# colinsongf/keyword_spotting

Hardware: AMD Instinct MI355X
Metric: mel-frames/s (real-time 10 ms-hop audio streams sustained = value/100) (higher is better)
Workload: dtype f32

## Files before the change

keyword_spotting_amd/csrc/gru_device.h:

```cpp
#pragma once
#include <type_traits>

#include "kws_internal.h"

namespace kws {

typedef float f32x4 __attribute__((ext_vector_type(4)));

__device__ __forceinline__ f32x4 mfma4(float a, float b, f32x4 c) {
    return __builtin_amdgcn_mfma_f32_16x16x4f32(a, b, c, 0, 0, 0);
}
__device__ __forceinline__ float sigmoid_f(float x) {
    return __builtin_amdgcn_rcpf(1.0f + __expf(-x));
}
__device__ __forceinline__ float tanh_f(float x) {
    return 1.0f - 2.0f * __builtin_amdgcn_rcpf(1.0f + __expf(2.0f * x));
}
#define KWS_MFMA_A(acc, wa, bv) \
    asm volatile("v_mfma_f32_16x16x4_f32 %0, %1, %2, %0" : "+v"(acc) : "a"(wa), "v"(bv))
__device__ __forceinline__ void mfma_fence(f32x4& a, f32x4& b, f32x4& c, f32x4& d) {
    asm volatile("s_nop 15" : "+v"(a), "+v"(b), "+v"(c), "+v"(d));
}
__device__ __forceinline__ void mfma_fence(f32x4& a, f32x4& b) {
    asm volatile("s_nop 15" : "+v"(a), "+v"(b));
}
__device__ __forceinline__ void mfma_prefence(f32x4& a, f32x4& b, f32x4& c, f32x4& d) {
    asm volatile("s_nop 3" : "+v"(a), "+v"(b), "+v"(c), "+v"(d));
}
__device__ __forceinline__ void mfma_prefence(f32x4& a, f32x4& b) {
    asm volatile("s_nop 3" : "+v"(a), "+v"(b));
}
__device__ __forceinline__ f32x4 splat4(float v) { f32x4 r = {v, v, v, v}; return r; }
__device__ __forceinline__ float bitsel(unsigned m, float a, float b) {
    return __uint_as_float((__float_as_uint(a) & m) | (__float_as_uint(b) & ~m));
}
template <int I0, int I1, class F>
__device__ __forceinline__ void static_for(F&& f) {
    if constexpr (I0 < I1) {
        f(std::integral_constant<int, I0>{});
        static_for<I0 + 1, I1>(f);
    }
}
constexpr float kLog2e = 1.4426950408889634f;
typedef float f32x2 __attribute__((ext_vector_type(2)));
__device__ __forceinline__ f32x2 sigmoid2(f32x2 x) {
    const f32x2 t = x * -kLog2e;
    f32x2 e;
    e.x = __builtin_amdgcn_exp2f(t.x);
    e.y = __builtin_amdgcn_exp2f(t.y);
    const f32x2 d = e + 1.0f;
    f32x2 r;
    r.x = __builtin_amdgcn_rcpf(d.x);
    r.y = __builtin_amdgcn_rcpf(d.y);
#ifdef KWS_FAULT_INJECT
    r = r * 1.0078125f;
#endif
    return r;
}
__device__ __forceinline__ f32x2 tanh2(f32x2 x) {
    const f32x2 t = x * (2.0f * kLog2e);
    f32x2 e;
    e.x = __builtin_amdgcn_exp2f(t.x);
    e.y = __builtin_amdgcn_exp2f(t.y);
    const f32x2 d = e + 1.0f;
    f32x2 r;
    r.x = __builtin_amdgcn_rcpf(d.x);
    r.y = __builtin_amdgcn_rcpf(d.y);
    return r * -2.0f + 1.0f;
}
__device__ __forceinline__ f32x4 ld4(const float* p) { return *reinterpret_cast<const f32x4*>(p); }

__device__ __forceinline__ void lds_barrier() {
    asm volatile("s_waitcnt lgkmcnt(0)" ::: "memory");
    __builtin_amdgcn_s_barrier();
    asm volatile("" ::: "memory");
}
constexpr int kRingFrames = 16;
constexpr int xs_stride(int kcx) { return 4 * ((((kcx + 3) / 4) & 1) ? (kcx + 3) / 4 : (kcx + 3) / 4 + 1); }
struct EpilogueLds {
    float* pstage;
    float* lring;
    int* words;
    int* carry;
    int8_t* cwords;
};
constexpr size_t kEpilogueLdsBytes = (4 * 16 * 8 + kRingFrames * 16 * 8) * 4 + kRingFrames * 16 * 4 + 2 * 16 * 4;
__device__ __forceinline__ EpilogueLds epilogue_carve(char* base) {
    EpilogueLds e;
    e.pstage = reinterpret_cast<float*>(base);
    e.lring = e.pstage + 4 * 16 * 8;
    e.words = reinterpret_cast<int*>(e.lring + kRingFrames * 16 * 8);
    e.carry = e.words + kRingFrames * 16;
    e.cwords = nullptr;
    return e;
}

__device__ __forceinline__ void epilogue_fold(const EpilogueLds& e, int t, int lane) {
    if (lane < 32) {
        const int s = lane >> 1, half = lane & 1;
        f32x4 v = *reinterpret_cast<const f32x4*>(e.pstage + (0 * 16 + s) * 8 + 4 * half);
#pragma unroll
        for (int w = 1; w < 4; ++w) v += *reinterpret_cast<const f32x4*>(e.pstage + (w * 16 + s) * 8 + 4 * half);
        *reinterpret_cast<f32x4*>(e.lring + (((t & (kRingFrames - 1)) * 16 + s) * 8 + 4 * half)) = v;
    }
}

struct FoldRegs { f32x4 v[4]; };
__device__ __forceinline__ void epilogue_fold_load(const EpilogueLds& e, int lane, FoldRegs& r) {
    if (lane < 32) {
        const int s = lane >> 1, half = lane & 1;
#pragma unroll
        for (int w = 0; w < 4; ++w) r.v[w] = *reinterpret_cast<const f32x4*>(e.pstage + (w * 16 + s) * 8 + 4 * half);
    }
}
__device__ __forceinline__ void epilogue_fold_store(const EpilogueLds& e, int t, int lane, const FoldRegs& r) {
    if (lane < 32) {
        const int s = lane >> 1, half = lane & 1;
        const f32x4 v = ((r.v[0] + r.v[1]) + r.v[2]) + r.v[3];
        *reinterpret_cast<f32x4*>(e.lring + (((t & (kRingFrames - 1)) * 16 + s) * 8 + 4 * half)) = v;
    }
}

template <bool OPAQUE_LANE = false>
__device__ __forceinline__ void epilogue_flush(const GruLayerParams& p, const EpilogueLds& e, int group, int t0,
                                               int n, int w, int lane, bool final_flush) {
    if constexpr (OPAQUE_LANE) asm volatile("" : "+v"(lane));
    const int f = 4 * w + (lane & 3);
    const int s = lane >> 2;
    const int b = group * kStreamsPerGroup + s;
    const int C = p.C;
    float lg[kMaxClasses];
    {
        const f32x4* row = reinterpret_cast<const f32x4*>(e.lring + (f * 16 + s) * 8);
        const f32x4 lo = row[0], hi = row[1];
#pragma unroll
        for (int c = 0; c < 4; ++c) { lg[c] = lo[c]; lg[4 + c] = hi[c]; }
    }
    if (p.use_relu) {
#pragma unroll
        for (int c = 0; c < kMaxClasses; ++c) {
            lg[c] = fmaxf(lg[c], 0.f);
            if (p.value_clip > 0.f) lg[c] = fminf(lg[c], 20.f);
        }
    }
    float m = lg[0];
#pragma unroll
    for (int c = 1; c < kMaxClasses; ++c) m = (c < C) ? fmaxf(m, lg[c]) : m;
    float pr[kMaxClasses];
    float sum = 0.f;
#pragma unroll
    for (int c = 0; c < kMaxClasses; ++c) {
        pr[c] = (c < C) ? __expf(lg[c] - m) : 0.f;
        sum += pr[c];
    }
    const float inv = __builtin_amdgcn_rcpf(sum);
#pragma unroll
    for (int c = 0; c < kMaxClasses; ++c) pr[c] *= inv;
    int word = -1;
    float best = -1.f;
#pragma unroll
    for (int c = 1; c < kMaxClasses - 1; ++c) {
        if (c < C - 1 && pr[c] > best) { best = pr[c]; word = c - 1; }
    }
    if (!(best > p.decode_thres)) word = -1;
    e.words[f * 16 + s] = word;
    if (e.cwords != nullptr) {
        int ln = lane;
        asm volatile("" : "+v"(ln));
        const int f2 = 4 * w + (ln & 3);
        if (f2 < n) e.cwords[(ln >> 2) * kWinTailWordsStride + t0 + f2] = (int8_t)word;
    }
    const bool mine = b < p.B && f < n;
    const size_t row = (size_t)b * (p.t_stride ? p.t_stride : p.T) + (t0 + f);
    if (mine) {
        if (C == 6) {
            if (p.logits) {
                float2* o = reinterpret_cast<float2*>(p.logits + row * 6);
                o[0] = make_float2(lg[0], lg[1]); o[1] = make_float2(lg[2], lg[3]); o[2] = make_float2(lg[4], lg[5]);
            }
            if (p.softmax) {
                float2* o = reinterpret_cast<float2*>(p.softmax + row * 6);
                o[0] = make_float2(pr[0], pr[1]); o[1] = make_float2(pr[2], pr[3]); o[2] = make_float2(pr[4], pr[5]);
            }
        } else {
            if (p.logits) {
#pragma unroll
                for (int c = 0; c < kMaxClasses; ++c)
                    if (c < C) p.logits[row * C + c] = lg[c];
            }
            if (p.softmax) {
#pragma unroll
                for (int c = 0; c < kMaxClasses; ++c)
                    if (c < C) p.softmax[row * C + c] = pr[c];
            }
        }
    }
    lds_barrier();
    const int blk = (t0 / kRingFrames) & 1;
    const int prev = f == 0 ? e.carry[blk * 16 + s] : e.words[(f - 1) * 16 + s];
    const int token = (word >= 0 && word != prev) ? word + 1 : 0;
    if (f == n - 1) {
        if (!final_flush) e.carry[(blk ^ 1) * 16 + s] = word;
        else if (b < p.B && p.prev_word) p.prev_word[b] = word;
    }
    if (mine && p.tokens) p.tokens[row] = (int8_t)token;
}


}
```

keyword_spotting_amd/csrc/gru_kernels.hip:

```cpp
#include <cstddef>

#include "gru_device.h"
#include "launch.h"
#include "window_device.h"

namespace kws {

template <int KCX, bool FIRST, bool LAST, bool WINDOW = false>
__global__ void __launch_bounds__(256) __attribute__((amdgpu_waves_per_eu(1, 1)))
gru_layer_resident(const GruLayerParams p) {
    static_assert(!WINDOW || (LAST && !FIRST), "the window tail belongs to the last layer of a stack");
    constexpr int H = 128, NT = 8, KCH = 32;
    const int tid = threadIdx.x;
    const int w = __builtin_amdgcn_readfirstlane(tid >> 6);
    const int lane = tid & 63, g = lane >> 4, s = lane & 15;
    const int n_groups = (p.B + kStreamsPerGroup - 1) / kStreamsPerGroup;
    int group = blockIdx.x;
    int b_raw = group * kStreamsPerGroup + s;
    bool bvalid = b_raw < p.B;
    int b = bvalid ? b_raw : p.B - 1;
    const int T = p.T;
    const int n0 = 2 * w, n1 = 2 * w + 1;

    extern __shared__ __attribute__((aligned(16))) char smem[];
    f32x4* hbuf = reinterpret_cast<f32x4*>(smem);
    f32x4* rhbuf = hbuf + NT * 64;
    f32x4* wlds = rhbuf + NT * 64;
    EpilogueLds epi = epilogue_carve(reinterpret_cast<char*>(wlds + 4 * KCX * 64));
    if constexpr (WINDOW) epi.cwords = reinterpret_cast<int8_t*>(reinterpret_cast<char*>(wlds + 4 * KCX * 64) + kEpilogueLdsBytes);
    const uint8_t* win_dl = reinterpret_cast<const uint8_t*>(epi.cwords) + 16 * kWinTailWordsStride;
    constexpr size_t kWinOffset = offsetof(GruLayerParams, win);
    if constexpr (WINDOW) window_tail_prepare(window_tail_params_from_kernarg(kWinOffset), const_cast<uint8_t*>(win_dl), tid);
    constexpr int kXsStride = xs_stride(KCX);
    float* xs = reinterpret_cast<float*>(reinterpret_cast<char*>(wlds + 4 * KCX * 64) + (LAST ? kEpilogueLdsBytes : 0));

    float wgh[2][2][KCH];
    float wch[2][KCH];
    float wcx[2][KCX];
    const f32x4* wh4 = reinterpret_cast<const f32x4*>(p.wh);
#pragma unroll
    for (int j = 0; j < 2; ++j) {
        const int n = 2 * w + j;
#pragma unroll
        for (int k4 = 0; k4 < KCH / 4; ++k4) {
            const f32x4 vr = wh4[((n * 3 + 0) * (KCH / 4) + k4) * 64 + lane];
            const f32x4 vu = wh4[((n * 3 + 1) * (KCH / 4) + k4) * 64 + lane];
            const f32x4 vc = wh4[((n * 3 + 2) * (KCH / 4) + k4) * 64 + lane];
#pragma unroll
            for (int e = 0; e < 4; ++e) {
                wgh[j][0][4 * k4 + e] = vr[e];
                wgh[j][1][4 * k4 + e] = vu[e];
                wch[j][4 * k4 + e] = vc[e];
            }
        }
    }
    if constexpr (FIRST) {
#pragma unroll
        for (int j = 0; j < 2; ++j)
#pragma unroll
            for (int kc = 0; kc < KCX; ++kc) wcx[j][kc] = p.wx[(((2 * w + j) * 3 + 2) * KCX + kc) * 64 + lane];
        for (int kc = 0; kc < KCX; ++kc) {
            f32x4 v;
            v.x = p.wx[((n0 * 3 + 0) * KCX + kc) * 64 + lane];
            v.y = p.wx[((n0 * 3 + 1) * KCX + kc) * 64 + lane];
            v.z = p.wx[((n1 * 3 + 0) * KCX + kc) * 64 + lane];
            v.w = p.wx[((n1 * 3 + 1) * KCX + kc) * 64 + lane];
            wlds[(w * KCX + kc) * 64 + lane] = v;
        }
    } else {
        const f32x4* wx4 = reinterpret_cast<const f32x4*>(p.wx);
#pragma unroll
        for (int j = 0; j < 2; ++j)
#pragma unroll
            for (int k4 = 0; k4 < KCX / 4; ++k4) {
                const f32x4 vc = wx4[(((2 * w + j) * 3 + 2) * (KCX / 4) + k4) * 64 + lane];
#pragma unroll
                for (int e = 0; e < 4; ++e) wcx[j][4 * k4 + e] = vc[e];
            }
        for (int k4 = 0; k4 < KCX / 4; ++k4) {
            const f32x4 r0 = wx4[((n0 * 3 + 0) * (KCX / 4) + k4) * 64 + lane];
            const f32x4 u0 = wx4[((n0 * 3 + 1) * (KCX / 4) + k4) * 64 + lane];
            const f32x4 r1 = wx4[((n1 * 3 + 0) * (KCX / 4) + k4) * 64 + lane];
            const f32x4 u1 = wx4[((n1 * 3 + 1) * (KCX / 4) + k4) * 64 + lane];
#pragma unroll
            for (int e = 0; e < 4; ++e)
                wlds[(w * KCX + 4 * k4 + e) * 64 + lane] = (f32x4){r0[e], u0[e], r1[e], u1[e]};
        }
    }
#pragma unroll
    for (int j = 0; j < 2; ++j) {
#pragma unroll
        for (int kc = 0; kc < KCH; ++kc) {
            asm volatile("" : "+a"(wgh[j][0][kc]));
            asm volatile("" : "+a"(wgh[j][1][kc]));
            asm volatile("" : "+a"(wch[j][kc]));
        }
    }
    asm volatile("s_nop 7" ::: "memory");
    f32x4 bias_r[2], bias_u[2], bias_c[2];
#pragma unroll
    for (int j = 0; j < 2; ++j) {
        const int n = 2 * w + j;
        bias_r[j] = ld4(p.bias + 0 * H + n * 16 + 4 * g);
        bias_u[j] = ld4(p.bias + 1 * H + n * 16 + 4 * g);
        bias_c[j] = ld4(p.bias + 2 * H + n * 16 + 4 * g);
    }
    float wfc[2][4];
    f32x4 bfc4 = splat4(0.f);
    if (LAST) {
#pragma unroll
        for (int j = 0; j < 2; ++j)
#pragma unroll
            for (int e = 0; e < 4; ++e) wfc[j][e] = p.wfc[((2 * w + j) * 4 + e) * 64 + lane];
        if (w == 0) bfc4 = ld4(p.bfc + 4 * g);
    }

    int len_s = T;
    f32x4 hreg[2];
    const float4* xl_src = nullptr;
    const float4* xprev = nullptr;
    constexpr int XQ = KCX;
    const int xl_row = lane / XQ, xl_q = lane % XQ;
    const bool xl_active = FIRST && lane < 4 * XQ;
    auto enter_group = [&]() {
        b_raw = group * kStreamsPerGroup + s;
        bvalid = b_raw < p.B;
        b = bvalid ? b_raw : p.B - 1;
        const bool do_reset = p.reset != nullptr && p.reset[b] != 0;
        len_s = p.seq_len ? p.seq_len[b] - p.t_base : T;
#pragma unroll
        for (int j = 0; j < 2; ++j) {
            const int n = 2 * w + j;
            hreg[j] = do_reset ? splat4(0.f) : ld4(p.state_in + (size_t)b * H + n * 16 + 4 * g);
            hbuf[n * 64 + lane] = hreg[j];
        }
        if (LAST && tid < 16) {
            const int bb = group * kStreamsPerGroup + tid;
            int pw = -1;
            if (bb < p.B && p.prev_word && !(p.reset && p.reset[bb])) pw = p.prev_word[bb];
            epi.carry[tid] = pw;
        }
        if constexpr (FIRST) {
            const int xl_b = min(group * kStreamsPerGroup + 4 * w + (xl_active ? xl_row : 0), p.B - 1);
            xl_src = reinterpret_cast<const float4*>(p.x_mel + (size_t)xl_b * (p.t_stride ? p.t_stride : T) * p.I) + xl_q;
        } else {
            xprev = p.x_prev + (size_t)group * T * NT * 64 + lane;
        }
    };

    float4 xl_inflight = make_float4(0.f, 0.f, 0.f, 0.f);
    auto coop_issue = [&](int t_req) {
        const int t = t_req < T ? t_req : T - 1;
        if (xl_active) xl_inflight = xl_src[(size_t)t * XQ];
    };
    auto coop_commit = [&]() {
        if (xl_active) {
            float* dst = xs + (4 * (4 * w + xl_row)) * kXsStride + xl_q;
            dst[0 * kXsStride] = xl_inflight.x;
            dst[1 * kXsStride] = xl_inflight.y;
            dst[2 * kXsStride] = xl_inflight.z;
            dst[3 * kXsStride] = xl_inflight.w;
        }
    };
    float xbuf0[KCX];
    auto read_xs = [&](float (&dst)[KCX]) {
        const float* row = xs + (4 * s + g) * kXsStride;
#pragma unroll
        for (int k4 = 0; k4 < KCX / 4; ++k4) {
            const f32x4 v = *reinterpret_cast<const f32x4*>(row + 4 * k4);
            dst[4 * k4 + 0] = v[0]; dst[4 * k4 + 1] = v[1]; dst[4 * k4 + 2] = v[2]; dst[4 * k4 + 3] = v[3];
        }
        if constexpr (KCX % 4 >= 2) {
            const f32x2 v = *reinterpret_cast<const f32x2*>(row + (KCX / 4) * 4);
            dst[(KCX / 4) * 4 + 0] = v[0]; dst[(KCX / 4) * 4 + 1] = v[1];
        }
        if constexpr (KCX % 2 == 1) dst[KCX - 1] = row[KCX - 1];
    };
    auto load_x_slice = [&](float (&dst)[KCX], int t_req, const int sl) {
        if constexpr (!FIRST) {
            const int t = t_req < T ? t_req : T - 1;
            const float4 v = xprev[((size_t)t * NT + sl) * 64];
            dst[4 * sl + 0] = v.x; dst[4 * sl + 1] = v.y; dst[4 * sl + 2] = v.z; dst[4 * sl + 3] = v.w;
        }
    };

    f32x4 acc_r[2], acc_u[2], acc_c[2];
    auto gates_x_part = [&](const float (&xB)[KCX], auto k0_, auto k1_, auto pin_) {
        constexpr int K0 = decltype(k0_)::value, K1 = decltype(k1_)::value;
        constexpr bool PIN = decltype(pin_)::value;
        f32x4 ring[3];
        if (K0 < K1) ring[K0 % 3] = wlds[(w * KCX + K0) * 64 + lane];
        if (K0 + 1 < K1) ring[(K0 + 1) % 3] = wlds[(w * KCX + K0 + 1) * 64 + lane];
#pragma unroll
        for (int kc = K0; kc < K1; ++kc) {
            if (kc + 2 < K1) ring[(kc + 2) % 3] = wlds[(w * KCX + kc + 2) * 64 + lane];
            if (PIN) __builtin_amdgcn_sched_barrier(0);
            const f32x4 a4 = ring[kc % 3];
            acc_r[0] = mfma4(a4.x, xB[kc], acc_r[0]);
            acc_u[0] = mfma4(a4.y, xB[kc], acc_u[0]);
            acc_r[1] = mfma4(a4.z, xB[kc], acc_r[1]);
            acc_u[1] = mfma4(a4.w, xB[kc], acc_u[1]);
            if (PIN) __builtin_amdgcn_sched_barrier(0);
        }
    };
    using pinned = std::true_type;
    constexpr int KSPLIT = KCX / 2;
    using k_lo = std::integral_constant<int, 0>;
    using k_mid = std::integral_constant<int, KSPLIT>;
    using k_hi = std::integral_constant<int, KCX>;
    auto cand_x = [&](const float (&xB)[KCX]) {
#pragma unroll
        for (int j = 0; j < 2; ++j) acc_c[j] = bias_c[j];
#pragma unroll
        for (int kc = 0; kc < KCX; ++kc) {
            acc_c[0] = mfma4(wcx[0][kc], xB[kc], acc_c[0]);
            acc_c[1] = mfma4(wcx[1][kc], xB[kc], acc_c[1]);
        }
    };

    f32x4 hb_a, hb_b;

    auto frame = [&](int t, float (&xcur)[KCX], float (&xnxt)[KCX]) {
        mfma_prefence(acc_r[0], acc_u[0], acc_r[1], acc_u[1]);
#pragma unroll
        for (int nn = 0; nn < NT; ++nn) {
            const f32x4 hb = (nn & 1) ? hb_b : hb_a;
            if (nn + 2 < NT) {
                if (nn & 1) hb_b = hbuf[(nn + 2) * 64 + lane]; else hb_a = hbuf[(nn + 2) * 64 + lane];
            }
            if constexpr (FIRST) { if (nn == 0) coop_issue(t + 2); } else load_x_slice(xnxt, t + 1, nn);
            __builtin_amdgcn_sched_barrier(0);
#pragma unroll
            for (int e = 0; e < 4; ++e) {
                const int kc = 4 * nn + e;
                const float hv = hb[e];
                KWS_MFMA_A(acc_r[0], wgh[0][0][kc], hv);
                KWS_MFMA_A(acc_u[0], wgh[0][1][kc], hv);
                KWS_MFMA_A(acc_r[1], wgh[1][0][kc], hv);
                KWS_MFMA_A(acc_u[1], wgh[1][1][kc], hv);
            }
        }
        mfma_fence(acc_r[0], acc_u[0], acc_r[1], acc_u[1]);
        if constexpr (FIRST) read_xs(xcur);
        f32x4 u[2];
#pragma unroll
        for (int j = 0; j < 2; ++j) {
            const f32x2 r_lo = sigmoid2((f32x2){acc_r[j][0], acc_r[j][1]});
            const f32x2 r_hi = sigmoid2((f32x2){acc_r[j][2], acc_r[j][3]});
            const f32x2 rh_lo = r_lo * (f32x2){hreg[j][0], hreg[j][1]};
            const f32x2 rh_hi = r_hi * (f32x2){hreg[j][2], hreg[j][3]};
            rhbuf[(2 * w + j) * 64 + lane] = (f32x4){rh_lo.x, rh_lo.y, rh_hi.x, rh_hi.y};
        }
#pragma unroll
        for (int j = 0; j < 2; ++j) {
            const f32x2 u_lo = sigmoid2((f32x2){acc_u[j][0], acc_u[j][1]});
            const f32x2 u_hi = sigmoid2((f32x2){acc_u[j][2], acc_u[j][3]});
            u[j] = (f32x4){u_lo.x, u_lo.y, u_hi.x, u_hi.y};
        }
#pragma unroll
        for (int j = 0; j < 2; ++j) { acc_r[j] = bias_r[j]; acc_u[j] = bias_u[j]; }
        __builtin_amdgcn_sched_barrier(0);
        gates_x_part(xcur, k_lo{}, k_mid{}, pinned{});
        lds_barrier();
        hb_a = rhbuf[0 * 64 + lane];
        hb_b = rhbuf[1 * 64 + lane];
        gates_x_part(xcur, k_mid{}, k_hi{}, pinned{});

        mfma_prefence(acc_c[0], acc_c[1]);
#pragma unroll
        for (int nn = 0; nn < NT; ++nn) {
            const f32x4 rb = (nn & 1) ? hb_b : hb_a;
            if (nn + 2 < NT) {
                if (nn & 1) hb_b = rhbuf[(nn + 2) * 64 + lane]; else hb_a = rhbuf[(nn + 2) * 64 + lane];
            }
            __builtin_amdgcn_sched_barrier(0);
#pragma unroll
            for (int e = 0; e < 4; ++e) {
                const int kc = 4 * nn + e;
                const float rv = rb[e];
                KWS_MFMA_A(acc_c[0], wch[0][kc], rv);
                KWS_MFMA_A(acc_c[1], wch[1][kc], rv);
            }
        }
        mfma_fence(acc_c[0], acc_c[1]);
        const unsigned live = t < len_s ? 0xffffffffu : 0u;
        f32x4 hout[2];
#pragma unroll
        for (int j = 0; j < 2; ++j) {
#pragma unroll
            for (int h2 = 0; h2 < 2; ++h2) {
                const f32x2 c = tanh2((f32x2){acc_c[j][2 * h2], acc_c[j][2 * h2 + 1]});
                const f32x2 uu = {u[j][2 * h2], u[j][2 * h2 + 1]};
                const f32x2 hh = {hreg[j][2 * h2], hreg[j][2 * h2 + 1]};
                const f32x2 hn = (1.0f - uu) * c + uu * hh;
                hreg[j][2 * h2] = bitsel(live, hn.x, hh.x);
                hreg[j][2 * h2 + 1] = bitsel(live, hn.y, hh.y);
                if (LAST) {
                    hout[j][2 * h2] = bitsel(live, hn.x, 0.f);
                    hout[j][2 * h2 + 1] = bitsel(live, hn.y, 0.f);
                }
            }
        }
#pragma unroll
        for (int j = 0; j < 2; ++j) acc_c[j] = bias_c[j];
        constexpr int NCX = 2 * KCX;
        constexpr int NPOST = NCX >= 32 ? 16 : 8;
        constexpr int NPRE = NCX - NPOST;
        auto cand_x_mfma = [&](auto mc) {
            constexpr int m = decltype(mc)::value, kc = m / 2;
            if constexpr (m % 2 == 0) acc_c[0] = mfma4(wcx[0][kc], xcur[kc], acc_c[0]);
            else acc_c[1] = mfma4(wcx[1][kc], xcur[kc], acc_c[1]);
        };
        if constexpr (FIRST) coop_commit();
#pragma unroll
        for (int j = 0; j < 2; ++j) {
            hbuf[(2 * w + j) * 64 + lane] = hreg[j];
            if (!LAST) {
                const f32x4 o = hreg[j];
                p.h_out[((size_t)group * T + t) * NT * 64 + (2 * w + j) * 64 + lane] =
                    make_float4(o[0], o[1], o[2], o[3]);
            }
        }
        if (LAST) {
            f32x4 accf = bfc4;
#pragma unroll
            for (int j = 0; j < 2; ++j)
#pragma unroll
                for (int e = 0; e < 4; ++e) accf = mfma4(wfc[j][e], hout[j][e], accf);
            if (g < 2) *reinterpret_cast<f32x4*>(epi.pstage + (w * 16 + s) * 8 + 4 * g) = accf;
        }
        __builtin_amdgcn_sched_barrier(0);
        static_for<0, NPRE>(cand_x_mfma);
        __builtin_amdgcn_sched_barrier(0);
        lds_barrier();
        hb_a = hbuf[0 * 64 + lane];
        hb_b = hbuf[1 * 64 + lane];
        FoldRegs fold;
        const bool folder = LAST && w == (t & 3);
        if (folder) epilogue_fold_load(epi, lane, fold);
        __builtin_amdgcn_sched_barrier(0);
        static_for<NPRE, NCX>(cand_x_mfma);
        __builtin_amdgcn_sched_barrier(0);
        if (LAST) {
            if (folder) epilogue_fold_store(epi, t, lane, fold);
            if (((t + 1) & (kRingFrames - 1)) == 0 || t == T - 1) {
                const int t0 = t & ~(kRingFrames - 1);
                lds_barrier();
                epilogue_flush(p, epi, group, t0, t - t0 + 1, w, lane, t == T - 1);
            }
        }
    };

    for (; group < n_groups; group += gridDim.x) {
    enter_group();
    __syncthreads();
    if (T > 0) {
        if constexpr (FIRST) {
            coop_issue(0);
            coop_commit();
            __syncthreads();
            read_xs(xbuf0);
            coop_issue(1);
        } else {
#pragma unroll
            for (int sl = 0; sl < NT; ++sl) load_x_slice(xbuf0, 0, sl);
        }
#pragma unroll
        for (int j = 0; j < 2; ++j) { acc_r[j] = bias_r[j]; acc_u[j] = bias_u[j]; }
        gates_x_part(xbuf0, k_lo{}, k_hi{}, pinned{});
        hb_a = hbuf[0 * 64 + lane];
        hb_b = hbuf[1 * 64 + lane];
        cand_x(xbuf0);
        if constexpr (FIRST) {
            __syncthreads();
            coop_commit();
            __syncthreads();
        }
    }
    for (int t = 0; t < T; ++t) frame(t, xbuf0, xbuf0);

    if (bvalid) {
#pragma unroll
        for (int j = 0; j < 2; ++j)
            *reinterpret_cast<f32x4*>(p.state_out + (size_t)b * H + (2 * w + j) * 16 + 4 * g) = hreg[j];
    }
    __syncthreads();
    if constexpr (WINDOW) {
        const WindowTail win = window_tail_params_from_kernarg(kWinOffset);
        WindowTailRegs<2> wreq;
        window_tail_request<2>(win, p.B, group * kStreamsPerGroup, tid, wreq);
        window_tail<2>(win, p.B, group * kStreamsPerGroup, T, epi.cwords, kWinTailWordsStride, win_dl, reinterpret_cast<char*>(hbuf), tid, wreq);
        __syncthreads();
    }
    }
}

constexpr float kResidualScale = 0.7071067811865475f;
constexpr float kLayerNormEps = 1e-5f;

template <int TPW, bool FIRST, bool LAST, bool PIPE, bool WRAP = false>
__device__ __forceinline__ void gru_layer_generic_body(const GruLayerParams& p, const int group,
                                                       const GruWrapLayer& wl = GruWrapLayer{nullptr, 0.f, 0}) {
    constexpr int NT = 4 * TPW, H = 64 * TPW;
    const int tid = threadIdx.x;
    const int w = __builtin_amdgcn_readfirstlane(tid >> 6);
    const int lane = tid & 63, g = lane >> 4, s = lane & 15;
    const int b_raw = group * kStreamsPerGroup + s;
    const bool bvalid = b_raw < p.B;
    const int b = bvalid ? b_raw : p.B - 1;
    const int T = p.T, I = p.I;
    const int KCX4 = p.KCX / 4;

    extern __shared__ __attribute__((aligned(16))) char smem[];
    f32x4* hbuf = reinterpret_cast<f32x4*>(smem);
    f32x4* rhbuf = hbuf + NT * 64;
    f32x4* xstage = rhbuf + NT * 64;
    f32x4* biasl = xstage + NT * 64;
    const EpilogueLds epi = epilogue_carve(reinterpret_cast<char*>(biasl + 3 * NT * 4));
    f32x4* const xln = WRAP ? reinterpret_cast<f32x4*>(reinterpret_cast<char*>(biasl + 3 * NT * 4) + kEpilogueLdsBytes) : nullptr;
    const bool w_ln = WRAP && wl.igamma != nullptr;
    const bool w_res = WRAP && !FIRST && wl.residual != 0;
    const bool w_staged = w_ln || w_res;

    const __amdgpu_buffer_rsrc_t wx_rsrc = __builtin_amdgcn_make_buffer_rsrc(const_cast<float*>(p.wx), (short)0, 0x7fffffff, 0x00020000);
    const __amdgpu_buffer_rsrc_t wh_rsrc = __builtin_amdgcn_make_buffer_rsrc(const_cast<float*>(p.wh), (short)0, 0x7fffffff, 0x00020000);
    const int lane16 = lane * 16;
    auto bload = [&](const __amdgpu_buffer_rsrc_t& r, int frag) -> f32x4 {
        return __builtin_bit_cast(f32x4, __builtin_amdgcn_raw_buffer_load_b128(r, lane16, frag * 1024, 0));
    };

    f32x4 hreg[TPW];
    const bool do_reset = p.reset != nullptr && p.reset[b] != 0;
    const int len_s = p.seq_len ? p.seq_len[b] - p.t_base : T;
    for (int i = tid; i < 3 * NT * 4; i += 256) biasl[i] = ld4(p.bias + 4 * i);
#pragma unroll
    for (int j = 0; j < TPW; ++j) {
        const int n = TPW * w + j;
        hreg[j] = do_reset ? splat4(0.f) : ld4(p.state_in + (size_t)b * H + n * 16 + 4 * g);
        hbuf[n * 64 + lane] = hreg[j];
    }
    f32x4 bfc4 = splat4(0.f);
    if (LAST) {
        if (w == 0) bfc4 = ld4(p.bfc + 4 * g);
        if (tid < 16) {
            const int bb = group * kStreamsPerGroup + tid;
            int pw = -1;
            if (bb < p.B && p.prev_word && !(p.reset && p.reset[bb])) pw = p.prev_word[bb];
            epi.carry[tid] = pw;
        }
    }
    const float* xrow = FIRST ? p.x_mel + (size_t)b * (p.t_stride ? p.t_stride : T) * I : nullptr;
    const __amdgpu_buffer_rsrc_t xp_rsrc = __builtin_amdgcn_make_buffer_rsrc(
        FIRST ? const_cast<float*>(p.wh) : const_cast<float*>(reinterpret_cast<const float*>(p.x_prev + (size_t)group * T * NT * 64)),
        (short)0, 0x7fffffff, 0x00020000);
    const __amdgpu_buffer_rsrc_t ho_rsrc = __builtin_amdgcn_make_buffer_rsrc(
        LAST ? const_cast<float*>(p.wh) : reinterpret_cast<float*>(p.h_out + (size_t)group * T * NT * 64), (short)0, 0x7fffffff, 0x00020000);
    constexpr int kSysScope = 1 | 16;
    const bool vec_ok = (I & 3) == 0;
    __syncthreads();

    auto x_operand = [&](int t, int k4) -> f32x4 {
        f32x4 xb;
        if (WRAP && w_staged) {
            xb = (w_ln ? xln : xstage)[k4 * 64 + lane];
        } else if (FIRST) {
            const int k = 16 * k4 + 4 * g;
            const float* src = xrow + (size_t)t * I + k;
            if (vec_ok && k + 3 < I) {
                xb = ld4(src);
            } else {
#pragma unroll
                for (int e = 0; e < 4; ++e) xb[e] = (k + e < I) ? src[e] : 0.f;
            }
        } else if (PIPE) {
            xb = xstage[k4 * 64 + lane];
        } else {
            xb = bload(xp_rsrc, t * NT + k4);
        }
        return xb;
    };
    constexpr int RT = TPW, NP = TPW / RT;
    struct RowX { f32x4 a[RT][3]; f32x4 xb; };
    struct RowH { f32x4 a[RT][2]; };
    struct RowC { f32x4 a[RT]; };
    auto load_x = [&](RowX& r, int t, int q) {
        const int qq = q < KCX4 * NP ? q : KCX4 * NP - 1, kk = qq / NP, part = qq - kk * NP;
#pragma unroll
        for (int j = 0; j < RT; ++j)
#pragma unroll
            for (int c = 0; c < 3; ++c) r.a[j][c] = bload(wx_rsrc, ((TPW * w + part * RT + j) * 3 + c) * KCX4 + kk);
        r.xb = x_operand(t, kk);
        __builtin_amdgcn_sched_barrier(0);
    };
    auto load_h = [&](RowH& r, int q) {
        const int qq = q < NT * NP ? q : NT * NP - 1, kk = qq / NP, part = qq - kk * NP;
#pragma unroll
        for (int j = 0; j < RT; ++j)
#pragma unroll
            for (int c = 0; c < 2; ++c) r.a[j][c] = bload(wh_rsrc, ((TPW * w + part * RT + j) * 3 + c) * NT + kk);
        __builtin_amdgcn_sched_barrier(0);
    };
    auto load_c = [&](RowC& r, int q) {
        const int qq = q < NT * NP ? q : NT * NP - 1, kk = qq / NP, part = qq - kk * NP;
#pragma unroll
        for (int j = 0; j < RT; ++j) r.a[j] = bload(wh_rsrc, ((TPW * w + part * RT + j) * 3 + 2) * NT + kk);
        __builtin_amdgcn_sched_barrier(0);
    };
    auto mel_operand = [&](int t, int k4) -> f32x4 {
        f32x4 xb;
        const int k = 16 * k4 + 4 * g;
        const float* src = xrow + (size_t)t * I + k;
        if (vec_ok && k + 3 < I) {
            xb = ld4(src);
        } else {
#pragma unroll
            for (int e = 0; e < 4; ++e) xb[e] = (k + e < I) ? src[e] : 0.f;
        }
        return xb;
    };
    auto wrap_frame = [&](int t) {
        f32x4* const raw = FIRST ? xln : xstage;
        if (FIRST) {
            for (int k0 = w; k0 < KCX4; k0 += 16) {
                f32x4 v[4];
#pragma unroll
                for (int i = 0; i < 4; ++i) if (k0 + 4 * i < KCX4) v[i] = mel_operand(t, k0 + 4 * i);
#pragma unroll
                for (int i = 0; i < 4; ++i) if (k0 + 4 * i < KCX4) raw[(k0 + 4 * i) * 64 + lane] = v[i];
            }
            __syncthreads();
        } else if (!PIPE) {
            f32x4 v[NT / 4];
#pragma unroll
            for (int i = 0; i < NT / 4; ++i) v[i] = bload(xp_rsrc, t * NT + w + 4 * i);
#pragma unroll
            for (int i = 0; i < NT / 4; ++i) raw[(w + 4 * i) * 64 + lane] = v[i];
            __syncthreads();
        }
        if (!w_ln) return;
        float sum = 0.f;
        for (int k4 = 0; k4 < KCX4; ++k4) {
            const f32x4 v = raw[k4 * 64 + lane];
            sum += (v[0] + v[1]) + (v[2] + v[3]);
        }
        sum += __shfl_xor(sum, 16);
        sum += __shfl_xor(sum, 32);
        const float mu = sum / (float)I;
        float sq = 0.f;
        for (int k4 = 0; k4 < KCX4; ++k4) {
            const f32x4 v = raw[k4 * 64 + lane];
#pragma unroll
            for (int e = 0; e < 4; ++e) {
                float d = v[e] - mu;
                if (FIRST) d = (16 * k4 + 4 * g + e < I) ? d : 0.f;
                sq = fmaf(d, d, sq);
            }
        }
        sq += __shfl_xor(sq, 16);
        sq += __shfl_xor(sq, 32);
        const float scale = wl.ibeta * rsqrtf(sq / (float)I + kLayerNormEps);
        if (FIRST) __syncthreads();
        for (int k0 = w; k0 < KCX4; k0 += 16) {
            f32x4 gm[4];
#pragma unroll
            for (int i = 0; i < 4; ++i) if (k0 + 4 * i < KCX4) gm[i] = ld4(wl.igamma + 16 * (k0 + 4 * i) + 4 * g);
#pragma unroll
            for (int i = 0; i < 4; ++i) {
                const int k4 = k0 + 4 * i;
                if (k4 < KCX4) {
                    const f32x4 v = raw[k4 * 64 + lane];
                    f32x4 o;
#pragma unroll
                    for (int e = 0; e < 4; ++e) {
                        o[e] = fmaf(v[e] - mu, scale, gm[i][e]);
                        if (FIRST) o[e] = (16 * k4 + 4 * g + e < I) ? o[e] : 0.f;
                    }
                    xln[k4 * 64 + lane] = o;
                }
            }
        }
        __syncthreads();
    };
    for (int t = 0; t < T; ++t) {
        f32x4 acc_r[TPW], acc_u[TPW], acc_c[TPW];
#pragma unroll
        for (int j = 0; j < TPW; ++j) {
            const int n = TPW * w + j;
            acc_r[j] = biasl[(0 * NT + n) * 4 + g]; acc_u[j] = biasl[(1 * NT + n) * 4 + g]; acc_c[j] = biasl[(2 * NT + n) * 4 + g];
        }
        if (PIPE && !FIRST) {
            int spins = 0;
            while (__hip_atomic_load(p.ready_in + group, __ATOMIC_RELAXED, __HIP_MEMORY_SCOPE_AGENT) <= t) {
                __builtin_amdgcn_s_sleep(2);
                if (++spins > (1 << 24)) { if (lane == 0) *reinterpret_cast<volatile int*>(p.pipe_error) = 1; break; }
            }
            asm volatile("" ::: "memory");
            f32x4 xv[NT / 4];
#pragma unroll
            for (int i = 0; i < NT / 4; ++i)
                xv[i] = __builtin_bit_cast(f32x4, __builtin_amdgcn_raw_buffer_load_b128(xp_rsrc, lane16, (t * NT + (w + 4 * i)) * 1024, kSysScope));
#pragma unroll
            for (int i = 0; i < NT / 4; ++i) xstage[(w + 4 * i) * 64 + lane] = xv[i];
            __syncthreads();
        }
        if constexpr (WRAP) {
            if (w_staged) wrap_frame(t);
        }
        {
#define KWS_MMA_X(P_)                                                                                 \
            _Pragma("unroll") for (int j = 0; j < RT; ++j)                                             \
                _Pragma("unroll") for (int e = 0; e < 4; ++e) {                                        \
                    acc_r[P_ * RT + j] = mfma4(rr.a[j][0][e], rr.xb[e], acc_r[P_ * RT + j]);           \
                    acc_u[P_ * RT + j] = mfma4(rr.a[j][1][e], rr.xb[e], acc_u[P_ * RT + j]);           \
                    acc_c[P_ * RT + j] = mfma4(rr.a[j][2][e], rr.xb[e], acc_c[P_ * RT + j]);           \
                }
            RowX ra, rb;
            const int NQ = KCX4 * NP;
            load_x(ra, t, 0);
#pragma nounroll
            for (int q = 0; q < NQ; q += 2) {
                load_x(rb, t, q + 1);
                { const RowX& rr = ra; KWS_MMA_X(0); __builtin_amdgcn_sched_barrier(0); }
                if (q + 1 < NQ) {
                    load_x(ra, t, q + 2);
                    { const RowX& rr = rb; if (NP == 2) { KWS_MMA_X((NP - 1)); } else { KWS_MMA_X(0); } __builtin_amdgcn_sched_barrier(0); }
                }
            }
#undef KWS_MMA_X
        }
        {
#define KWS_MMA_H(P_)                                                                                 \
            _Pragma("unroll") for (int j = 0; j < RT; ++j)                                             \
                _Pragma("unroll") for (int e = 0; e < 4; ++e) {                                        \
                    acc_r[P_ * RT + j] = mfma4(rr.a[j][0][e], hb[e], acc_r[P_ * RT + j]);              \
                    acc_u[P_ * RT + j] = mfma4(rr.a[j][1][e], hb[e], acc_u[P_ * RT + j]);              \
                }
            RowH ra, rb;
            constexpr int NQ = NT * NP;
            load_h(ra, 0);
#pragma nounroll
            for (int q = 0; q < NQ; q += 2) {
                load_h(rb, q + 1);
                { const RowH& rr = ra; const f32x4 hb = hbuf[(q / NP) * 64 + lane]; KWS_MMA_H(0); __builtin_amdgcn_sched_barrier(0); }
                load_h(ra, q + 2);
                { const RowH& rr = rb; const f32x4 hb = hbuf[((q + 1) / NP) * 64 + lane];
                  if (NP == 2) { KWS_MMA_H((NP - 1)); } else { KWS_MMA_H(0); } __builtin_amdgcn_sched_barrier(0); }
            }
#undef KWS_MMA_H
        }
        f32x4 u[TPW];
#pragma unroll
        for (int j = 0; j < TPW; ++j) {
            f32x4 rh;
#pragma unroll
            for (int e = 0; e < 4; ++e) {
                rh[e] = sigmoid_f(acc_r[j][e]) * hreg[j][e];
                u[j][e] = sigmoid_f(acc_u[j][e]);
            }
            rhbuf[(TPW * w + j) * 64 + lane] = rh;
        }
        RowC ca, cb;
        if (PIPE && !LAST) asm volatile("s_waitcnt vmcnt(0)" ::: "memory");
        load_c(ca, 0);
        __syncthreads();
        if (PIPE && !LAST && t > 0 && tid == 0)
            __hip_atomic_store(p.ready_out + group, t, __ATOMIC_RELAXED, __HIP_MEMORY_SCOPE_AGENT);
        {
#define KWS_MMA_C(P_)                                                                                 \
            _Pragma("unroll") for (int j = 0; j < RT; ++j)                                             \
                _Pragma("unroll") for (int e = 0; e < 4; ++e)                                          \
                    acc_c[P_ * RT + j] = mfma4(rr.a[j][e], rb[e], acc_c[P_ * RT + j]);
            constexpr int NQ = NT * NP;
#pragma nounroll
            for (int q = 0; q < NQ; q += 2) {
                load_c(cb, q + 1);
                { const RowC& rr = ca; const f32x4 rb = rhbuf[(q / NP) * 64 + lane]; KWS_MMA_C(0); __builtin_amdgcn_sched_barrier(0); }
                load_c(ca, q + 2);
                { const RowC& rr = cb; const f32x4 rb = rhbuf[((q + 1) / NP) * 64 + lane];
                  if (NP == 2) { KWS_MMA_C((NP - 1)); } else { KWS_MMA_C(0); } __builtin_amdgcn_sched_barrier(0); }
            }
#undef KWS_MMA_C
        }
        const unsigned live = t < len_s ? 0xffffffffu : 0u;
        f32x4 accf = bfc4;
#pragma unroll
        for (int j = 0; j < TPW; ++j) {
            const int n = TPW * w + j;
            f32x4 hout;
            f32x4 xr = splat4(0.f), seam = splat4(0.f);
            if (WRAP && w_res) xr = xstage[n * 64 + lane];
#pragma unroll
            for (int e = 0; e < 4; ++e) {
                const float c = tanh_f(acc_c[j][e]);
                const float hn = fmaf(u[j][e], hreg[j][e], (1.0f - u[j][e]) * c);
                hreg[j][e] = bitsel(live, hn, hreg[j][e]);
                hout[e] = bitsel(live, hn, 0.f);
                if (WRAP) {
                    const float o = w_res ? kResidualScale * (hn + xr[e]) : hn;
                    hout[e] = bitsel(live, o, 0.f);
                    seam[e] = bitsel(live, o, hreg[j][e]);
                }
            }
            hbuf[n * 64 + lane] = hreg[j];
            if (!LAST) {
                const f32x4 o = WRAP ? seam : hreg[j];
                float4* dst = p.h_out + ((size_t)group * T + t) * NT * 64 + n * 64 + lane;
                if (PIPE) {
                    typedef int i32x4 __attribute__((ext_vector_type(4)));
                    __builtin_amdgcn_raw_buffer_store_b128(__builtin_bit_cast(i32x4, o), ho_rsrc, lane16, (t * NT + n) * 1024, kSysScope);
                } else {
                    *dst = make_float4(o[0], o[1], o[2], o[3]);
                }
            } else {
#pragma unroll
                for (int e = 0; e < 4; ++e) accf = mfma4(p.wfc[(n * 4 + e) * 64 + lane], hout[e], accf);
            }
        }
        if (LAST && g < 2) *reinterpret_cast<f32x4*>(epi.pstage + (w * 16 + s) * 8 + 4 * g) = accf;
        __syncthreads();
        if (LAST) {
            if (w == (t & 3)) epilogue_fold(epi, t, lane);
            if (((t + 1) & (kRingFrames - 1)) == 0 || t == T - 1) {
                const int t0 = t & ~(kRingFrames - 1);
                __syncthreads();
                epilogue_flush(p, epi, group, t0, t - t0 + 1, w, lane, t == T - 1);
            }
        }
    }
    if (PIPE && !LAST) {
        asm volatile("s_waitcnt vmcnt(0)" ::: "memory");
        __syncthreads();
        if (tid == 0) __hip_atomic_store(p.ready_out + group, T, __ATOMIC_RELAXED, __HIP_MEMORY_SCOPE_AGENT);
    }
    if (bvalid) {
#pragma unroll
        for (int j = 0; j < TPW; ++j)
            *reinterpret_cast<f32x4*>(p.state_out + (size_t)b * H + (TPW * w + j) * 16 + 4 * g) = hreg[j];
    }
}

template <int TPW, bool FIRST, bool LAST>
__global__ void __launch_bounds__(256) gru_layer_generic(const GruLayerParams p) {
    gru_layer_generic_body<TPW, FIRST, LAST, false>(p, blockIdx.x);
}

template <int TPW>
__global__ void __launch_bounds__(256) gru_stack_generic_pipelined(const GruStackParams sp) {
    int layer, group;
    if (sp.xcd_affine) {
        const int xcd = blockIdx.x & 7, slot = blockIdx.x >> 3, per = 8 / sp.L;
        layer = xcd % sp.L;
        group = slot * per + xcd / sp.L;
        if (group >= sp.G) return;
    } else {
        layer = blockIdx.x / sp.G;
        group = blockIdx.x - layer * sp.G;
    }
    if (layer == 0) gru_layer_generic_body<TPW, true, false, true>(sp.layer[0], group);
    else if (layer == sp.L - 1) gru_layer_generic_body<TPW, false, true, true>(sp.layer[layer], group);
    else gru_layer_generic_body<TPW, false, false, true>(sp.layer[layer], group);
}

template <int TPW, bool FIRST, bool LAST>
__global__ void __launch_bounds__(256) gru_layer_generic_wrapped(const GruLayerParams p, const GruWrapLayer wl) {
    gru_layer_generic_body<TPW, FIRST, LAST, false, true>(p, blockIdx.x, wl);
}
template <int TPW>
__global__ void __launch_bounds__(256) gru_stack_generic_pipelined_wrapped(const GruStackParams sp, const GruWrapParams wp) {
    int layer, group;
    if (sp.xcd_affine) {
        const int xcd = blockIdx.x & 7, slot = blockIdx.x >> 3, per = 8 / sp.L;
        layer = xcd % sp.L;
        group = slot * per + xcd / sp.L;
        if (group >= sp.G) return;
    } else {
        layer = blockIdx.x / sp.G;
        group = blockIdx.x - layer * sp.G;
    }
    if (layer == 0) gru_layer_generic_body<TPW, true, false, true, true>(sp.layer[0], group, wp.layer[0]);
    else if (layer == sp.L - 1) gru_layer_generic_body<TPW, false, true, true, true>(sp.layer[layer], group, wp.layer[layer]);
    else gru_layer_generic_body<TPW, false, false, true, true>(sp.layer[layer], group, wp.layer[layer]);
}
static_assert(sizeof(GruStackParams) + sizeof(GruWrapParams) <= 4096, "kernel arguments");

static size_t resident_lds_bytes(int kcx, bool first, bool last) {
    size_t n = 2 * 8 * 64 * 16 + (size_t)4 * kcx * 64 * 16;
    if (last) n += kEpilogueLdsBytes;
    if (first) n += (size_t)64 * xs_stride(kcx) * 4;
    return n;
}
static size_t generic_lds_bytes(int hidden, bool last) {
    size_t n = (size_t)3 * (hidden / 16) * 64 * 16 + (size_t)3 * hidden * 4;
    if (last) n += kEpilogueLdsBytes;
    return n;
}

int gru_resident_kcx(int in_dim, bool first) { return first ? (in_dim + 3) / 4 : 32; }

bool gru_resident_supported(int hidden, int in_dim, bool first) {
    if (hidden != 128) return false;
    if (!first) return in_dim == 128;
    return in_dim == 32 || in_dim == 40 || in_dim == 48 || in_dim == 60 || in_dim == 64;
}

bool gru_resident_takes_window(bool first, bool last) { return last && !first; }

hipError_t launch_gru_layer_resident(const GruLayerParams& p, bool first, bool last, hipStream_t st) {
    const size_t lds = resident_lds_bytes(p.KCX, first, last);
    const dim3 grid(persistent_grid(p.B));
    if (p.win.tab != nullptr) {
        if (!gru_resident_takes_window(first, last) || p.seq_len) return hipErrorInvalidValue;
        return launch_lds<gru_layer_resident<32, false, true, true>>(grid, dim3(256), lds + kWinTailWordsBytes, st, p);
    }
    return with_bool(last, [&](auto la) {
        if (!first) return launch_lds<gru_layer_resident<32, false, la()>>(grid, dim3(256), lds, st, p);
        return with_int<8, 10, 12, 15, 16>(p.KCX, [&](auto kcx) {
            return launch_lds<gru_layer_resident<kcx(), true, la()>>(grid, dim3(256), lds, st, p);
        });
    });
}

hipError_t launch_gru_stack_generic_pipelined(const GruStackParams& sp, int hidden, hipStream_t st) {
    const size_t lds = one_workgroup_per_cu(generic_lds_bytes(hidden, true));
    const dim3 grid(pipelined_grid(sp.L, sp.G, sp.xcd_affine));
    return with_tpw<1, 2, 4>(hidden, [&](auto tpw) {
        return launch_lds<gru_stack_generic_pipelined<tpw()>>(grid, dim3(256), lds, st, sp);
    });
}

hipError_t launch_gru_layer_generic(const GruLayerParams& p, int hidden, bool first, bool last,
                                    hipStream_t st) {
    size_t lds = generic_lds_bytes(hidden, last);
    if (p.t_stride != 0) lds = one_workgroup_per_cu(lds);
    return with_layer_shape<1, 2, 4>(hidden, first, last, [&](auto tpw, auto fi, auto la) {
        return launch_lds<gru_layer_generic<tpw(), fi(), la()>>(dim3(groups_of(p.B)), dim3(256), lds, st, p);
    });
}

hipError_t launch_gru_layer_generic_wrapped(const GruLayerParams& p, const GruWrapLayer& wl, int hidden, bool first, bool last,
                                            hipStream_t st) {
    size_t lds = generic_lds_bytes(hidden, true) + gru_wrapped_extra_lds(p.KCX / 4);
    if (p.t_stride != 0) lds = one_workgroup_per_cu(lds);
    return with_layer_shape<1, 2, 4>(hidden, first, last, [&](auto tpw, auto fi, auto la) {
        return launch_lds<gru_layer_generic_wrapped<tpw(), fi(), la()>>(dim3(groups_of(p.B)), dim3(256), lds, st, p, wl);
    });
}

hipError_t launch_gru_stack_generic_pipelined_wrapped(const GruStackParams& sp, const GruWrapParams& wp, int hidden, hipStream_t st) {
    int kx4 = 0;
    for (int l = 0; l < sp.L; ++l) kx4 = sp.layer[l].KCX / 4 > kx4 ? sp.layer[l].KCX / 4 : kx4;
    const size_t lds = one_workgroup_per_cu(generic_lds_bytes(hidden, true) + gru_wrapped_extra_lds(kx4));
    const dim3 grid(pipelined_grid(sp.L, sp.G, sp.xcd_affine));
    return with_tpw<1, 2, 4>(hidden, [&](auto tpw) {
        return launch_lds<gru_stack_generic_pipelined_wrapped<tpw()>>(grid, dim3(256), lds, st, sp, wp);
    });
}

}
```

Baseline: 390.1 million.

## Move resident GRU kernel to own file with group-cooperative x prefetch

```diff
diff --git a/keyword_spotting_amd/csrc/gru_device.h b/keyword_spotting_amd/csrc/gru_device.h
--- a/keyword_spotting_amd/csrc/gru_device.h
+++ b/keyword_spotting_amd/csrc/gru_device.h
@@ -16,8 +16,12 @@
 __device__ __forceinline__ float tanh_f(float x) {
     return 1.0f - 2.0f * __builtin_amdgcn_rcpf(1.0f + __expf(2.0f * x));
 }
+#if KWS_RESIDENT_VGPR_FORM
+#define KWS_MFMA_A(acc, wa, bv) acc = mfma4(wa, bv, acc)
+#else
 #define KWS_MFMA_A(acc, wa, bv) \
     asm volatile("v_mfma_f32_16x16x4_f32 %0, %1, %2, %0" : "+v"(acc) : "a"(wa), "v"(bv))
+#endif
 __device__ __forceinline__ void mfma_fence(f32x4& a, f32x4& b, f32x4& c, f32x4& d) {
     asm volatile("s_nop 15" : "+v"(a), "+v"(b), "+v"(c), "+v"(d));
 }
diff --git a/keyword_spotting_amd/csrc/gru_kernels.hip b/keyword_spotting_amd/csrc/gru_kernels.hip
--- a/keyword_spotting_amd/csrc/gru_kernels.hip
+++ b/keyword_spotting_amd/csrc/gru_kernels.hip
@@ -5,395 +5,6 @@
 #include "window_device.h"
 
 namespace kws {
-
-template <int KCX, bool FIRST, bool LAST, bool WINDOW = false>
-__global__ void __launch_bounds__(256) __attribute__((amdgpu_waves_per_eu(1, 1)))
-gru_layer_resident(const GruLayerParams p) {
-    static_assert(!WINDOW || (LAST && !FIRST), "the window tail belongs to the last layer of a stack");
-    constexpr int H = 128, NT = 8, KCH = 32;
-    const int tid = threadIdx.x;
-    const int w = __builtin_amdgcn_readfirstlane(tid >> 6);
-    const int lane = tid & 63, g = lane >> 4, s = lane & 15;
-    const int n_groups = (p.B + kStreamsPerGroup - 1) / kStreamsPerGroup;
-    int group = blockIdx.x;
-    int b_raw = group * kStreamsPerGroup + s;
-    bool bvalid = b_raw < p.B;
-    int b = bvalid ? b_raw : p.B - 1;
-    const int T = p.T;
-    const int n0 = 2 * w, n1 = 2 * w + 1;
-
-    extern __shared__ __attribute__((aligned(16))) char smem[];
-    f32x4* hbuf = reinterpret_cast<f32x4*>(smem);
-    f32x4* rhbuf = hbuf + NT * 64;
-    f32x4* wlds = rhbuf + NT * 64;
-    EpilogueLds epi = epilogue_carve(reinterpret_cast<char*>(wlds + 4 * KCX * 64));
-    if constexpr (WINDOW) epi.cwords = reinterpret_cast<int8_t*>(reinterpret_cast<char*>(wlds + 4 * KCX * 64) + kEpilogueLdsBytes);
-    const uint8_t* win_dl = reinterpret_cast<const uint8_t*>(epi.cwords) + 16 * kWinTailWordsStride;
-    constexpr size_t kWinOffset = offsetof(GruLayerParams, win);
-    if constexpr (WINDOW) window_tail_prepare(window_tail_params_from_kernarg(kWinOffset), const_cast<uint8_t*>(win_dl), tid);
-    constexpr int kXsStride = xs_stride(KCX);
-    float* xs = reinterpret_cast<float*>(reinterpret_cast<char*>(wlds + 4 * KCX * 64) + (LAST ? kEpilogueLdsBytes : 0));
-
-    float wgh[2][2][KCH];
-    float wch[2][KCH];
-    float wcx[2][KCX];
-    const f32x4* wh4 = reinterpret_cast<const f32x4*>(p.wh);
-#pragma unroll
-    for (int j = 0; j < 2; ++j) {
-        const int n = 2 * w + j;
-#pragma unroll
-        for (int k4 = 0; k4 < KCH / 4; ++k4) {
-            const f32x4 vr = wh4[((n * 3 + 0) * (KCH / 4) + k4) * 64 + lane];
-            const f32x4 vu = wh4[((n * 3 + 1) * (KCH / 4) + k4) * 64 + lane];
-            const f32x4 vc = wh4[((n * 3 + 2) * (KCH / 4) + k4) * 64 + lane];
-#pragma unroll
-            for (int e = 0; e < 4; ++e) {
-                wgh[j][0][4 * k4 + e] = vr[e];
-                wgh[j][1][4 * k4 + e] = vu[e];
-                wch[j][4 * k4 + e] = vc[e];
-            }
-        }
-    }
-    if constexpr (FIRST) {
-#pragma unroll
-        for (int j = 0; j < 2; ++j)
-#pragma unroll
-            for (int kc = 0; kc < KCX; ++kc) wcx[j][kc] = p.wx[(((2 * w + j) * 3 + 2) * KCX + kc) * 64 + lane];
-        for (int kc = 0; kc < KCX; ++kc) {
-            f32x4 v;
-            v.x = p.wx[((n0 * 3 + 0) * KCX + kc) * 64 + lane];
-            v.y = p.wx[((n0 * 3 + 1) * KCX + kc) * 64 + lane];
-            v.z = p.wx[((n1 * 3 + 0) * KCX + kc) * 64 + lane];
-            v.w = p.wx[((n1 * 3 + 1) * KCX + kc) * 64 + lane];
-            wlds[(w * KCX + kc) * 64 + lane] = v;
-        }
-    } else {
-        const f32x4* wx4 = reinterpret_cast<const f32x4*>(p.wx);
-#pragma unroll
-        for (int j = 0; j < 2; ++j)
-#pragma unroll
-            for (int k4 = 0; k4 < KCX / 4; ++k4) {
-                const f32x4 vc = wx4[(((2 * w + j) * 3 + 2) * (KCX / 4) + k4) * 64 + lane];
-#pragma unroll
-                for (int e = 0; e < 4; ++e) wcx[j][4 * k4 + e] = vc[e];
-            }
-        for (int k4 = 0; k4 < KCX / 4; ++k4) {
-            const f32x4 r0 = wx4[((n0 * 3 + 0) * (KCX / 4) + k4) * 64 + lane];
-            const f32x4 u0 = wx4[((n0 * 3 + 1) * (KCX / 4) + k4) * 64 + lane];
-            const f32x4 r1 = wx4[((n1 * 3 + 0) * (KCX / 4) + k4) * 64 + lane];
-            const f32x4 u1 = wx4[((n1 * 3 + 1) * (KCX / 4) + k4) * 64 + lane];
-#pragma unroll
-            for (int e = 0; e < 4; ++e)
-                wlds[(w * KCX + 4 * k4 + e) * 64 + lane] = (f32x4){r0[e], u0[e], r1[e], u1[e]};
-        }
-    }
-#pragma unroll
-    for (int j = 0; j < 2; ++j) {
-#pragma unroll
-        for (int kc = 0; kc < KCH; ++kc) {
-            asm volatile("" : "+a"(wgh[j][0][kc]));
-            asm volatile("" : "+a"(wgh[j][1][kc]));
-            asm volatile("" : "+a"(wch[j][kc]));
-        }
-    }
-    asm volatile("s_nop 7" ::: "memory");
-    f32x4 bias_r[2], bias_u[2], bias_c[2];
-#pragma unroll
-    for (int j = 0; j < 2; ++j) {
-        const int n = 2 * w + j;
-        bias_r[j] = ld4(p.bias + 0 * H + n * 16 + 4 * g);
-        bias_u[j] = ld4(p.bias + 1 * H + n * 16 + 4 * g);
-        bias_c[j] = ld4(p.bias + 2 * H + n * 16 + 4 * g);
-    }
-    float wfc[2][4];
-    f32x4 bfc4 = splat4(0.f);
-    if (LAST) {
-#pragma unroll
-        for (int j = 0; j < 2; ++j)
-#pragma unroll
-            for (int e = 0; e < 4; ++e) wfc[j][e] = p.wfc[((2 * w + j) * 4 + e) * 64 + lane];
-        if (w == 0) bfc4 = ld4(p.bfc + 4 * g);
-    }
-
-    int len_s = T;
-    f32x4 hreg[2];
-    const float4* xl_src = nullptr;
-    const float4* xprev = nullptr;
-    constexpr int XQ = KCX;
-    const int xl_row = lane / XQ, xl_q = lane % XQ;
-    const bool xl_active = FIRST && lane < 4 * XQ;
-    auto enter_group = [&]() {
-        b_raw = group * kStreamsPerGroup + s;
-        bvalid = b_raw < p.B;
-        b = bvalid ? b_raw : p.B - 1;
-        const bool do_reset = p.reset != nullptr && p.reset[b] != 0;
-        len_s = p.seq_len ? p.seq_len[b] - p.t_base : T;
-#pragma unroll
-        for (int j = 0; j < 2; ++j) {
-            const int n = 2 * w + j;
-            hreg[j] = do_reset ? splat4(0.f) : ld4(p.state_in + (size_t)b * H + n * 16 + 4 * g);
-            hbuf[n * 64 + lane] = hreg[j];
-        }
-        if (LAST && tid < 16) {
-            const int bb = group * kStreamsPerGroup + tid;
-            int pw = -1;
-            if (bb < p.B && p.prev_word && !(p.reset && p.reset[bb])) pw = p.prev_word[bb];
-            epi.carry[tid] = pw;
-        }
-        if constexpr (FIRST) {
-            const int xl_b = min(group * kStreamsPerGroup + 4 * w + (xl_active ? xl_row : 0), p.B - 1);
-            xl_src = reinterpret_cast<const float4*>(p.x_mel + (size_t)xl_b * (p.t_stride ? p.t_stride : T) * p.I) + xl_q;
-        } else {
-            xprev = p.x_prev + (size_t)group * T * NT * 64 + lane;
-        }
-    };
-
-    float4 xl_inflight = make_float4(0.f, 0.f, 0.f, 0.f);
-    auto coop_issue = [&](int t_req) {
-        const int t = t_req < T ? t_req : T - 1;
-        if (xl_active) xl_inflight = xl_src[(size_t)t * XQ];
-    };
-    auto coop_commit = [&]() {
-        if (xl_active) {
-            float* dst = xs + (4 * (4 * w + xl_row)) * kXsStride + xl_q;
-            dst[0 * kXsStride] = xl_inflight.x;
-            dst[1 * kXsStride] = xl_inflight.y;
-            dst[2 * kXsStride] = xl_inflight.z;
-            dst[3 * kXsStride] = xl_inflight.w;
-        }
-    };
-    float xbuf0[KCX];
-    auto read_xs = [&](float (&dst)[KCX]) {
-        const float* row = xs + (4 * s + g) * kXsStride;
-#pragma unroll
-        for (int k4 = 0; k4 < KCX / 4; ++k4) {
-            const f32x4 v = *reinterpret_cast<const f32x4*>(row + 4 * k4);
-            dst[4 * k4 + 0] = v[0]; dst[4 * k4 + 1] = v[1]; dst[4 * k4 + 2] = v[2]; dst[4 * k4 + 3] = v[3];
-        }
-        if constexpr (KCX % 4 >= 2) {
-            const f32x2 v = *reinterpret_cast<const f32x2*>(row + (KCX / 4) * 4);
-            dst[(KCX / 4) * 4 + 0] = v[0]; dst[(KCX / 4) * 4 + 1] = v[1];
-        }
-        if constexpr (KCX % 2 == 1) dst[KCX - 1] = row[KCX - 1];
-    };
-    auto load_x_slice = [&](float (&dst)[KCX], int t_req, const int sl) {
-        if constexpr (!FIRST) {
-            const int t = t_req < T ? t_req : T - 1;
-            const float4 v = xprev[((size_t)t * NT + sl) * 64];
-            dst[4 * sl + 0] = v.x; dst[4 * sl + 1] = v.y; dst[4 * sl + 2] = v.z; dst[4 * sl + 3] = v.w;
-        }
-    };
-
-    f32x4 acc_r[2], acc_u[2], acc_c[2];
-    auto gates_x_part = [&](const float (&xB)[KCX], auto k0_, auto k1_, auto pin_) {
-        constexpr int K0 = decltype(k0_)::value, K1 = decltype(k1_)::value;
-        constexpr bool PIN = decltype(pin_)::value;
-        f32x4 ring[3];
-        if (K0 < K1) ring[K0 % 3] = wlds[(w * KCX + K0) * 64 + lane];
-        if (K0 + 1 < K1) ring[(K0 + 1) % 3] = wlds[(w * KCX + K0 + 1) * 64 + lane];
-#pragma unroll
-        for (int kc = K0; kc < K1; ++kc) {
-            if (kc + 2 < K1) ring[(kc + 2) % 3] = wlds[(w * KCX + kc + 2) * 64 + lane];
-            if (PIN) __builtin_amdgcn_sched_barrier(0);
-            const f32x4 a4 = ring[kc % 3];
-            acc_r[0] = mfma4(a4.x, xB[kc], acc_r[0]);
-            acc_u[0] = mfma4(a4.y, xB[kc], acc_u[0]);
-            acc_r[1] = mfma4(a4.z, xB[kc], acc_r[1]);
-            acc_u[1] = mfma4(a4.w, xB[kc], acc_u[1]);
-            if (PIN) __builtin_amdgcn_sched_barrier(0);
-        }
-    };
-    using pinned = std::true_type;
-    constexpr int KSPLIT = KCX / 2;
-    using k_lo = std::integral_constant<int, 0>;
-    using k_mid = std::integral_constant<int, KSPLIT>;
-    using k_hi = std::integral_constant<int, KCX>;
-    auto cand_x = [&](const float (&xB)[KCX]) {
-#pragma unroll
-        for (int j = 0; j < 2; ++j) acc_c[j] = bias_c[j];
-#pragma unroll
-        for (int kc = 0; kc < KCX; ++kc) {
-            acc_c[0] = mfma4(wcx[0][kc], xB[kc], acc_c[0]);
-            acc_c[1] = mfma4(wcx[1][kc], xB[kc], acc_c[1]);
-        }
-    };
-
-    f32x4 hb_a, hb_b;
-
-    auto frame = [&](int t, float (&xcur)[KCX], float (&xnxt)[KCX]) {
-        mfma_prefence(acc_r[0], acc_u[0], acc_r[1], acc_u[1]);
-#pragma unroll
-        for (int nn = 0; nn < NT; ++nn) {
-            const f32x4 hb = (nn & 1) ? hb_b : hb_a;
-            if (nn + 2 < NT) {
-                if (nn & 1) hb_b = hbuf[(nn + 2) * 64 + lane]; else hb_a = hbuf[(nn + 2) * 64 + lane];
-            }
-            if constexpr (FIRST) { if (nn == 0) coop_issue(t + 2); } else load_x_slice(xnxt, t + 1, nn);
-            __builtin_amdgcn_sched_barrier(0);
-#pragma unroll
-            for (int e = 0; e < 4; ++e) {
-                const int kc = 4 * nn + e;
-                const float hv = hb[e];
-                KWS_MFMA_A(acc_r[0], wgh[0][0][kc], hv);
-                KWS_MFMA_A(acc_u[0], wgh[0][1][kc], hv);
-                KWS_MFMA_A(acc_r[1], wgh[1][0][kc], hv);
-                KWS_MFMA_A(acc_u[1], wgh[1][1][kc], hv);
-            }
-        }
-        mfma_fence(acc_r[0], acc_u[0], acc_r[1], acc_u[1]);
-        if constexpr (FIRST) read_xs(xcur);
-        f32x4 u[2];
-#pragma unroll
-        for (int j = 0; j < 2; ++j) {
-            const f32x2 r_lo = sigmoid2((f32x2){acc_r[j][0], acc_r[j][1]});
-            const f32x2 r_hi = sigmoid2((f32x2){acc_r[j][2], acc_r[j][3]});
-            const f32x2 rh_lo = r_lo * (f32x2){hreg[j][0], hreg[j][1]};
-            const f32x2 rh_hi = r_hi * (f32x2){hreg[j][2], hreg[j][3]};
-            rhbuf[(2 * w + j) * 64 + lane] = (f32x4){rh_lo.x, rh_lo.y, rh_hi.x, rh_hi.y};
-        }
-#pragma unroll
-        for (int j = 0; j < 2; ++j) {
-            const f32x2 u_lo = sigmoid2((f32x2){acc_u[j][0], acc_u[j][1]});
-            const f32x2 u_hi = sigmoid2((f32x2){acc_u[j][2], acc_u[j][3]});
-            u[j] = (f32x4){u_lo.x, u_lo.y, u_hi.x, u_hi.y};
-        }
-#pragma unroll
-        for (int j = 0; j < 2; ++j) { acc_r[j] = bias_r[j]; acc_u[j] = bias_u[j]; }
-        __builtin_amdgcn_sched_barrier(0);
-        gates_x_part(xcur, k_lo{}, k_mid{}, pinned{});
-        lds_barrier();
-        hb_a = rhbuf[0 * 64 + lane];
-        hb_b = rhbuf[1 * 64 + lane];
-        gates_x_part(xcur, k_mid{}, k_hi{}, pinned{});
-
-        mfma_prefence(acc_c[0], acc_c[1]);
-#pragma unroll
-        for (int nn = 0; nn < NT; ++nn) {
-            const f32x4 rb = (nn & 1) ? hb_b : hb_a;
-            if (nn + 2 < NT) {
-                if (nn & 1) hb_b = rhbuf[(nn + 2) * 64 + lane]; else hb_a = rhbuf[(nn + 2) * 64 + lane];
-            }
-            __builtin_amdgcn_sched_barrier(0);
-#pragma unroll
-            for (int e = 0; e < 4; ++e) {
-                const int kc = 4 * nn + e;
-                const float rv = rb[e];
-                KWS_MFMA_A(acc_c[0], wch[0][kc], rv);
-                KWS_MFMA_A(acc_c[1], wch[1][kc], rv);
-            }
-        }
-        mfma_fence(acc_c[0], acc_c[1]);
-        const unsigned live = t < len_s ? 0xffffffffu : 0u;
-        f32x4 hout[2];
-#pragma unroll
-        for (int j = 0; j < 2; ++j) {
-#pragma unroll
-            for (int h2 = 0; h2 < 2; ++h2) {
-                const f32x2 c = tanh2((f32x2){acc_c[j][2 * h2], acc_c[j][2 * h2 + 1]});
-                const f32x2 uu = {u[j][2 * h2], u[j][2 * h2 + 1]};
-                const f32x2 hh = {hreg[j][2 * h2], hreg[j][2 * h2 + 1]};
-                const f32x2 hn = (1.0f - uu) * c + uu * hh;
-                hreg[j][2 * h2] = bitsel(live, hn.x, hh.x);
-                hreg[j][2 * h2 + 1] = bitsel(live, hn.y, hh.y);
-                if (LAST) {
-                    hout[j][2 * h2] = bitsel(live, hn.x, 0.f);
-                    hout[j][2 * h2 + 1] = bitsel(live, hn.y, 0.f);
-                }
-            }
-        }
-#pragma unroll
-        for (int j = 0; j < 2; ++j) acc_c[j] = bias_c[j];
-        constexpr int NCX = 2 * KCX;
-        constexpr int NPOST = NCX >= 32 ? 16 : 8;
-        constexpr int NPRE = NCX - NPOST;
-        auto cand_x_mfma = [&](auto mc) {
-            constexpr int m = decltype(mc)::value, kc = m / 2;
-            if constexpr (m % 2 == 0) acc_c[0] = mfma4(wcx[0][kc], xcur[kc], acc_c[0]);
-            else acc_c[1] = mfma4(wcx[1][kc], xcur[kc], acc_c[1]);
-        };
-        if constexpr (FIRST) coop_commit();
-#pragma unroll
-        for (int j = 0; j < 2; ++j) {
-            hbuf[(2 * w + j) * 64 + lane] = hreg[j];
-            if (!LAST) {
-                const f32x4 o = hreg[j];
-                p.h_out[((size_t)group * T + t) * NT * 64 + (2 * w + j) * 64 + lane] =
-                    make_float4(o[0], o[1], o[2], o[3]);
-            }
-        }
-        if (LAST) {
-            f32x4 accf = bfc4;
-#pragma unroll
-            for (int j = 0; j < 2; ++j)
-#pragma unroll
-                for (int e = 0; e < 4; ++e) accf = mfma4(wfc[j][e], hout[j][e], accf);
-            if (g < 2) *reinterpret_cast<f32x4*>(epi.pstage + (w * 16 + s) * 8 + 4 * g) = accf;
-        }
-        __builtin_amdgcn_sched_barrier(0);
-        static_for<0, NPRE>(cand_x_mfma);
-        __builtin_amdgcn_sched_barrier(0);
-        lds_barrier();
-        hb_a = hbuf[0 * 64 + lane];
-        hb_b = hbuf[1 * 64 + lane];
-        FoldRegs fold;
-        const bool folder = LAST && w == (t & 3);
-        if (folder) epilogue_fold_load(epi, lane, fold);
-        __builtin_amdgcn_sched_barrier(0);
-        static_for<NPRE, NCX>(cand_x_mfma);
-        __builtin_amdgcn_sched_barrier(0);
-        if (LAST) {
-            if (folder) epilogue_fold_store(epi, t, lane, fold);
-            if (((t + 1) & (kRingFrames - 1)) == 0 || t == T - 1) {
-                const int t0 = t & ~(kRingFrames - 1);
-                lds_barrier();
-                epilogue_flush(p, epi, group, t0, t - t0 + 1, w, lane, t == T - 1);
-            }
-        }
-    };
-
-    for (; group < n_groups; group += gridDim.x) {
-    enter_group();
-    __syncthreads();
-    if (T > 0) {
-        if constexpr (FIRST) {
-            coop_issue(0);
-            coop_commit();
-            __syncthreads();
-            read_xs(xbuf0);
-            coop_issue(1);
-        } else {
-#pragma unroll
-            for (int sl = 0; sl < NT; ++sl) load_x_slice(xbuf0, 0, sl);
-        }
-#pragma unroll
-        for (int j = 0; j < 2; ++j) { acc_r[j] = bias_r[j]; acc_u[j] = bias_u[j]; }
-        gates_x_part(xbuf0, k_lo{}, k_hi{}, pinned{});
-        hb_a = hbuf[0 * 64 + lane];
-        hb_b = hbuf[1 * 64 + lane];
-        cand_x(xbuf0);
-        if constexpr (FIRST) {
-            __syncthreads();
-            coop_commit();
-            __syncthreads();
-        }
-    }
-    for (int t = 0; t < T; ++t) frame(t, xbuf0, xbuf0);
-
-    if (bvalid) {
-#pragma unroll
-        for (int j = 0; j < 2; ++j)
-            *reinterpret_cast<f32x4*>(p.state_out + (size_t)b * H + (2 * w + j) * 16 + 4 * g) = hreg[j];
-    }
-    __syncthreads();
-    if constexpr (WINDOW) {
-        const WindowTail win = window_tail_params_from_kernarg(kWinOffset);
-        WindowTailRegs<2> wreq;
-        window_tail_request<2>(win, p.B, group * kStreamsPerGroup, tid, wreq);
-        window_tail<2>(win, p.B, group * kStreamsPerGroup, T, epi.cwords, kWinTailWordsStride, win_dl, reinterpret_cast<char*>(hbuf), tid, wreq);
-        __syncthreads();
-    }
-    }
-}
 
 constexpr float kResidualScale = 0.7071067811865475f;
 constexpr float kLayerNormEps = 1e-5f;
@@ -783,41 +394,10 @@
 }
 static_assert(sizeof(GruStackParams) + sizeof(GruWrapParams) <= 4096, "kernel arguments");
 
-static size_t resident_lds_bytes(int kcx, bool first, bool last) {
-    size_t n = 2 * 8 * 64 * 16 + (size_t)4 * kcx * 64 * 16;
-    if (last) n += kEpilogueLdsBytes;
-    if (first) n += (size_t)64 * xs_stride(kcx) * 4;
-    return n;
-}
 static size_t generic_lds_bytes(int hidden, bool last) {
     size_t n = (size_t)3 * (hidden / 16) * 64 * 16 + (size_t)3 * hidden * 4;
     if (last) n += kEpilogueLdsBytes;
     return n;
-}
-
-int gru_resident_kcx(int in_dim, bool first) { return first ? (in_dim + 3) / 4 : 32; }
-
-bool gru_resident_supported(int hidden, int in_dim, bool first) {
-    if (hidden != 128) return false;
-    if (!first) return in_dim == 128;
-    return in_dim == 32 || in_dim == 40 || in_dim == 48 || in_dim == 60 || in_dim == 64;
-}
-
-bool gru_resident_takes_window(bool first, bool last) { return last && !first; }
-
-hipError_t launch_gru_layer_resident(const GruLayerParams& p, bool first, bool last, hipStream_t st) {
-    const size_t lds = resident_lds_bytes(p.KCX, first, last);
-    const dim3 grid(persistent_grid(p.B));
-    if (p.win.tab != nullptr) {
-        if (!gru_resident_takes_window(first, last) || p.seq_len) return hipErrorInvalidValue;
-        return launch_lds<gru_layer_resident<32, false, true, true>>(grid, dim3(256), lds + kWinTailWordsBytes, st, p);
-    }
-    return with_bool(last, [&](auto la) {
-        if (!first) return launch_lds<gru_layer_resident<32, false, la()>>(grid, dim3(256), lds, st, p);
-        return with_int<8, 10, 12, 15, 16>(p.KCX, [&](auto kcx) {
-            return launch_lds<gru_layer_resident<kcx(), true, la()>>(grid, dim3(256), lds, st, p);
-        });
-    });
 }
 
 hipError_t launch_gru_stack_generic_pipelined(const GruStackParams& sp, int hidden, hipStream_t st) {
diff --git a/keyword_spotting_amd/csrc/gru_resident.hip b/keyword_spotting_amd/csrc/gru_resident.hip
--- /dev/null
+++ b/keyword_spotting_amd/csrc/gru_resident.hip
@@ -0,0 +1,496 @@
+#include <cstddef>
+
+#include "gru_device.h"
+#include "launch.h"
+#include "window_device.h"
+
+namespace kws {
+
+#if KWS_RESIDENT_VGPR_FORM
+template <class... A> __device__ __forceinline__ void resident_prefence(A&...) {}
+template <class... A> __device__ __forceinline__ void resident_fence(A&...) {}
+#else
+template <class... A> __device__ __forceinline__ void resident_prefence(A&... a) { mfma_prefence(a...); }
+template <class... A> __device__ __forceinline__ void resident_fence(A&... a) { mfma_fence(a...); }
+#endif
+
+
+constexpr int resident_kreg(bool first) { return first ? 0 : 2; }
+constexpr size_t resident_lds_bytes(int kcx, bool first, bool last) {
+    size_t n = 2 * 8 * 64 * 16 + (size_t)4 * (kcx - resident_kreg(first)) * 64 * 16;
+    if (!first) n += 8 * 64 * 16;
+    if (last) n += kEpilogueLdsBytes;
+    if (first) n += (size_t)64 * xs_stride(kcx) * 4;
+    return n;
+}
+
+template <int KCX, bool FIRST, bool LAST, bool WINDOW = false>
+__global__ void __launch_bounds__(256) __attribute__((amdgpu_waves_per_eu(1, 1)))
+gru_layer_resident(const GruLayerParams p) {
+    static_assert(!WINDOW || (LAST && !FIRST), "the window tail belongs to the last layer of a stack");
+    constexpr int H = 128, NT = 8, KCH = 32;
+    const int tid = threadIdx.x;
+    const int w = __builtin_amdgcn_readfirstlane(tid >> 6);
+    const int lane = tid & 63, g = lane >> 4, s = lane & 15;
+    const int n_groups = (p.B + kStreamsPerGroup - 1) / kStreamsPerGroup;
+    int group = blockIdx.x;
+    int b_raw = group * kStreamsPerGroup + s;
+    bool bvalid = b_raw < p.B;
+    int b = bvalid ? b_raw : p.B - 1;
+    const int T = p.T;
+    const int n0 = 2 * w, n1 = 2 * w + 1;
+
+    extern __shared__ __attribute__((aligned(16))) char smem[];
+    f32x4* hbuf = reinterpret_cast<f32x4*>(smem);
+    f32x4* rhbuf = hbuf + NT * 64;
+    constexpr int KREG = resident_kreg(FIRST), KL = KCX - KREG;
+    f32x4* wlds = rhbuf + NT * 64;
+    f32x4* xsb = wlds + 4 * KL * 64;
+    char* const lds_tail = reinterpret_cast<char*>(xsb + (FIRST ? 0 : NT * 64));
+    static_assert(resident_lds_bytes(KCX, FIRST, LAST) + (WINDOW ? kWinTailWordsBytes : 0) <= 160 * 1024, "LDS per CU");
+    EpilogueLds epi = epilogue_carve(lds_tail);
+    if constexpr (WINDOW) epi.cwords = reinterpret_cast<int8_t*>(lds_tail + kEpilogueLdsBytes);
+    const uint8_t* win_dl = reinterpret_cast<const uint8_t*>(epi.cwords) + 16 * kWinTailWordsStride;
+    constexpr size_t kWinOffset = offsetof(GruLayerParams, win);
+    if constexpr (WINDOW) window_tail_prepare(window_tail_params_from_kernarg(kWinOffset), const_cast<uint8_t*>(win_dl), tid);
+    constexpr int kXsStride = xs_stride(KCX);
+    float* xs = reinterpret_cast<float*>(lds_tail + (LAST ? kEpilogueLdsBytes : 0));
+
+    float wgh[2][2][KCH];
+    float wch[2][KCH];
+    float wcx[2][KCX];
+    float wgx[KREG ? KREG : 1][4];
+    const f32x4* wh4 = reinterpret_cast<const f32x4*>(p.wh);
+#pragma unroll
+    for (int j = 0; j < 2; ++j) {
+        const int n = 2 * w + j;
+#pragma unroll
+        for (int k4 = 0; k4 < KCH / 4; ++k4) {
+            const f32x4 vr = wh4[((n * 3 + 0) * (KCH / 4) + k4) * 64 + lane];
+            const f32x4 vu = wh4[((n * 3 + 1) * (KCH / 4) + k4) * 64 + lane];
+            const f32x4 vc = wh4[((n * 3 + 2) * (KCH / 4) + k4) * 64 + lane];
+#pragma unroll
+            for (int e = 0; e < 4; ++e) {
+                wgh[j][0][4 * k4 + e] = vr[e];
+                wgh[j][1][4 * k4 + e] = vu[e];
+                wch[j][4 * k4 + e] = vc[e];
+            }
+        }
+    }
+    if constexpr (FIRST) {
+#pragma unroll
+        for (int j = 0; j < 2; ++j)
+#pragma unroll
+            for (int kc = 0; kc < KCX; ++kc) wcx[j][kc] = p.wx[(((2 * w + j) * 3 + 2) * KCX + kc) * 64 + lane];
+        for (int kc = 0; kc < KCX; ++kc) {
+            f32x4 v;
+            v.x = p.wx[((n0 * 3 + 0) * KCX + kc) * 64 + lane];
+            v.y = p.wx[((n0 * 3 + 1) * KCX + kc) * 64 + lane];
+            v.z = p.wx[((n1 * 3 + 0) * KCX + kc) * 64 + lane];
+            v.w = p.wx[((n1 * 3 + 1) * KCX + kc) * 64 + lane];
+            wlds[(w * KL + kc) * 64 + lane] = v;
+        }
+    } else {
+        const f32x4* wx4 = reinterpret_cast<const f32x4*>(p.wx);
+#pragma unroll
+        for (int j = 0; j < 2; ++j)
+#pragma unroll
+            for (int k4 = 0; k4 < KCX / 4; ++k4) {
+                const f32x4 vc = wx4[(((2 * w + j) * 3 + 2) * (KCX / 4) + k4) * 64 + lane];
+#pragma unroll
+                for (int e = 0; e < 4; ++e) wcx[j][4 * k4 + e] = vc[e];
+            }
+        static_assert(KREG <= 4, "the register chunks come out of the first group of four");
+#pragma unroll
+        for (int k4 = 0; k4 < KCX / 4; ++k4) {
+            const f32x4 r0 = wx4[((n0 * 3 + 0) * (KCX / 4) + k4) * 64 + lane];
+            const f32x4 u0 = wx4[((n0 * 3 + 1) * (KCX / 4) + k4) * 64 + lane];
+            const f32x4 r1 = wx4[((n1 * 3 + 0) * (KCX / 4) + k4) * 64 + lane];
+            const f32x4 u1 = wx4[((n1 * 3 + 1) * (KCX / 4) + k4) * 64 + lane];
+#pragma unroll
+            for (int e = 0; e < 4; ++e) {
+                const f32x4 v = {r0[e], u0[e], r1[e], u1[e]};
+                if (e < KREG && k4 == 0) { wgx[e][0] = v[0]; wgx[e][1] = v[1]; wgx[e][2] = v[2]; wgx[e][3] = v[3]; }
+                if (e >= KREG || k4 != 0) wlds[(w * KL + 4 * k4 + e - KREG) * 64 + lane] = v;
+            }
+        }
+    }
+#pragma unroll
+    for (int j = 0; j < 2; ++j) {
+#pragma unroll
+        for (int kc = 0; kc < KCH; ++kc) {
+            asm volatile("" : "+a"(wgh[j][0][kc]));
+            asm volatile("" : "+a"(wgh[j][1][kc]));
+            asm volatile("" : "+a"(wch[j][kc]));
+        }
+    }
+#if KWS_RESIDENT_VGPR_FORM
+    if constexpr (KREG > 0) {
+#pragma unroll
+        for (int kc = 0; kc < KREG; ++kc)
+#pragma unroll
+            for (int e = 0; e < 4; ++e) asm volatile("" : "+a"(wgx[kc][e]));
+    }
+#endif
+    asm volatile("s_nop 7" ::: "memory");
+    f32x4 bias_r[2], bias_u[2], bias_c[2];
+#pragma unroll
+    for (int j = 0; j < 2; ++j) {
+        const int n = 2 * w + j;
+        bias_r[j] = ld4(p.bias + 0 * H + n * 16 + 4 * g);
+        bias_u[j] = ld4(p.bias + 1 * H + n * 16 + 4 * g);
+        bias_c[j] = ld4(p.bias + 2 * H + n * 16 + 4 * g);
+    }
+    float wfc[2][4];
+    f32x4 bfc4 = splat4(0.f);
+    if (LAST) {
+#pragma unroll
+        for (int j = 0; j < 2; ++j)
+#pragma unroll
+            for (int e = 0; e < 4; ++e) wfc[j][e] = p.wfc[((2 * w + j) * 4 + e) * 64 + lane];
+        if (w == 0) bfc4 = ld4(p.bfc + 4 * g);
+    }
+
+    int len_s = T;
+    f32x4 hreg[2];
+    const float4* xl_src = nullptr;
+    const float4* xprev = nullptr;
+    const float4* xg_next = nullptr;
+    constexpr int XQ = KCX;
+    const int xl_row = lane / XQ, xl_q = lane % XQ;
+    const bool xl_active = FIRST && lane < 4 * XQ;
+    auto enter_group = [&]() {
+        b_raw = group * kStreamsPerGroup + s;
+        bvalid = b_raw < p.B;
+        b = bvalid ? b_raw : p.B - 1;
+        const bool do_reset = p.reset != nullptr && p.reset[b] != 0;
+        len_s = p.seq_len ? p.seq_len[b] - p.t_base : T;
+#pragma unroll
+        for (int j = 0; j < 2; ++j) {
+            const int n = 2 * w + j;
+            hreg[j] = do_reset ? splat4(0.f) : ld4(p.state_in + (size_t)b * H + n * 16 + 4 * g);
+            hbuf[n * 64 + lane] = hreg[j];
+        }
+        if (LAST && tid < 16) {
+            const int bb = group * kStreamsPerGroup + tid;
+            int pw = -1;
+            if (bb < p.B && p.prev_word && !(p.reset && p.reset[bb])) pw = p.prev_word[bb];
+            epi.carry[tid] = pw;
+        }
+        if constexpr (FIRST) {
+            const int xl_b = min(group * kStreamsPerGroup + 4 * w + (xl_active ? xl_row : 0), p.B - 1);
+            xl_src = reinterpret_cast<const float4*>(p.x_mel + (size_t)xl_b * (p.t_stride ? p.t_stride : T) * p.I) + xl_q;
+        } else {
+            xprev = p.x_prev + (size_t)group * T * NT * 64 + lane;
+            xg_next = xprev + ((size_t)(1 < T ? 1 : 0) * NT + n0) * 64;
+        }
+    };
+
+    constexpr bool kIssueAtEnd = FIRST && !LAST;
+    float4 xl_inflight = make_float4(0.f, 0.f, 0.f, 0.f);
+    auto coop_issue = [&](int t_req) {
+        const int t = t_req < T ? t_req : T - 1;
+        if (xl_active) xl_inflight = xl_src[(size_t)t * XQ];
+    };
+    auto coop_commit = [&]() {
+        if (xl_active) {
+            float* dst = xs + (4 * (4 * w + xl_row)) * kXsStride + xl_q;
+            dst[0 * kXsStride] = xl_inflight.x;
+            dst[1 * kXsStride] = xl_inflight.y;
+            dst[2 * kXsStride] = xl_inflight.z;
+            dst[3 * kXsStride] = xl_inflight.w;
+        }
+    };
+    float xbuf0[KCX];
+    auto read_xs = [&](float (&dst)[KCX]) {
+        const float* row = xs + (4 * s + g) * kXsStride;
+#pragma unroll
+        for (int k4 = 0; k4 < KCX / 4; ++k4) {
+            const f32x4 v = *reinterpret_cast<const f32x4*>(row + 4 * k4);
+            dst[4 * k4 + 0] = v[0]; dst[4 * k4 + 1] = v[1]; dst[4 * k4 + 2] = v[2]; dst[4 * k4 + 3] = v[3];
+        }
+        if constexpr (KCX % 4 >= 2) {
+            const f32x2 v = *reinterpret_cast<const f32x2*>(row + (KCX / 4) * 4);
+            dst[(KCX / 4) * 4 + 0] = v[0]; dst[(KCX / 4) * 4 + 1] = v[1];
+        }
+        if constexpr (KCX % 2 == 1) dst[KCX - 1] = row[KCX - 1];
+    };
+    auto load_x_slice = [&](float (&dst)[KCX], int t_req, const int sl) {
+        if constexpr (!FIRST) {
+            const int t = t_req < T ? t_req : T - 1;
+            const float4 v = xprev[((size_t)t * NT + sl) * 64];
+            dst[4 * sl + 0] = v.x; dst[4 * sl + 1] = v.y; dst[4 * sl + 2] = v.z; dst[4 * sl + 3] = v.w;
+        }
+    };
+    float4 xg_inflight[2];
+    auto group_issue = [&](int t_req) {
+        if constexpr (!FIRST) {
+            xg_inflight[0] = xg_next[0];
+            xg_inflight[1] = xg_next[64];
+            if (t_req + 1 < T) xg_next += NT * 64;
+        }
+    };
+    auto group_commit = [&]() {
+        if constexpr (!FIRST) {
+#pragma unroll
+            for (int j = 0; j < 2; ++j)
+                xsb[(2 * w + j) * 64 + lane] = (f32x4){xg_inflight[j].x, xg_inflight[j].y, xg_inflight[j].z, xg_inflight[j].w};
+        }
+    };
+    auto read_x_slice = [&](float (&dst)[KCX], const int sl) {
+        if constexpr (!FIRST) {
+            const f32x4 v = xsb[sl * 64 + lane];
+            dst[4 * sl + 0] = v[0]; dst[4 * sl + 1] = v[1]; dst[4 * sl + 2] = v[2]; dst[4 * sl + 3] = v[3];
+        }
+    };
+
+    f32x4 acc_r[2], acc_u[2], acc_c[2];
+    auto gates_x_part = [&](const float (&xB)[KCX], auto k0_, auto k1_, auto pin_) {
+        constexpr int K0 = decltype(k0_)::value, K1 = decltype(k1_)::value;
+        constexpr bool PIN = decltype(pin_)::value;
+        constexpr int R0 = K0 < KREG ? KREG : K0;
+        f32x4 ring[3];
+        if (R0 < K1) ring[R0 % 3] = wlds[(w * KL + R0 - KREG) * 64 + lane];
+        if (R0 + 1 < K1) ring[(R0 + 1) % 3] = wlds[(w * KL + R0 + 1 - KREG) * 64 + lane];
+#pragma unroll
+        for (int kc = K0; kc < K1; ++kc) {
+            if (kc + 2 < K1 && kc + 2 >= R0 + 2) ring[(kc + 2) % 3] = wlds[(w * KL + kc + 2 - KREG) * 64 + lane];
+            if (PIN) __builtin_amdgcn_sched_barrier(0);
+            const int kr = kc < KREG ? kc : 0;
+            const f32x4 a4 = kc < KREG ? (f32x4){wgx[kr][0], wgx[kr][1], wgx[kr][2], wgx[kr][3]} : ring[kc % 3];
+            acc_r[0] = mfma4(a4.x, xB[kc], acc_r[0]);
+            acc_u[0] = mfma4(a4.y, xB[kc], acc_u[0]);
+            acc_r[1] = mfma4(a4.z, xB[kc], acc_r[1]);
+            acc_u[1] = mfma4(a4.w, xB[kc], acc_u[1]);
+            if (PIN) __builtin_amdgcn_sched_barrier(0);
+        }
+    };
+    using pinned = std::true_type;
+    constexpr int KSPLIT = KCX / 2;
+    using k_lo = std::integral_constant<int, 0>;
+    using k_mid = std::integral_constant<int, KSPLIT>;
+    using k_hi = std::integral_constant<int, KCX>;
+    auto cand_x = [&](const float (&xB)[KCX]) {
+#pragma unroll
+        for (int j = 0; j < 2; ++j) acc_c[j] = bias_c[j];
+#pragma unroll
+        for (int kc = 0; kc < KCX; ++kc) {
+            acc_c[0] = mfma4(wcx[0][kc], xB[kc], acc_c[0]);
+            acc_c[1] = mfma4(wcx[1][kc], xB[kc], acc_c[1]);
+        }
+    };
+
+    f32x4 hb_a, hb_b;
+
+    auto frame = [&](int t, float (&xcur)[KCX], float (&xnxt)[KCX]) {
+        resident_prefence(acc_r[0], acc_u[0], acc_r[1], acc_u[1]);
+#pragma unroll
+        for (int nn = 0; nn < NT; ++nn) {
+            const f32x4 hb = (nn & 1) ? hb_b : hb_a;
+            if (nn + 2 < NT) {
+                if (nn & 1) hb_b = hbuf[(nn + 2) * 64 + lane]; else hb_a = hbuf[(nn + 2) * 64 + lane];
+            }
+            if constexpr (FIRST) { if (!kIssueAtEnd && nn == 0) coop_issue(t + 2); }
+            else { if (nn == 0) group_issue(t + 2); read_x_slice(xnxt, nn); }
+            __builtin_amdgcn_sched_barrier(0);
+#pragma unroll
+            for (int e = 0; e < 4; ++e) {
+                const int kc = 4 * nn + e;
+                const float hv = hb[e];
+                KWS_MFMA_A(acc_r[0], wgh[0][0][kc], hv);
+                KWS_MFMA_A(acc_u[0], wgh[0][1][kc], hv);
+                KWS_MFMA_A(acc_r[1], wgh[1][0][kc], hv);
+                KWS_MFMA_A(acc_u[1], wgh[1][1][kc], hv);
+            }
+        }
+        resident_fence(acc_r[0], acc_u[0], acc_r[1], acc_u[1]);
+        if constexpr (FIRST) read_xs(xcur);
+        f32x4 u[2];
+#pragma unroll
+        for (int j = 0; j < 2; ++j) {
+            const f32x2 r_lo = sigmoid2((f32x2){acc_r[j][0], acc_r[j][1]});
+            const f32x2 r_hi = sigmoid2((f32x2){acc_r[j][2], acc_r[j][3]});
+            const f32x2 rh_lo = r_lo * (f32x2){hreg[j][0], hreg[j][1]};
+            const f32x2 rh_hi = r_hi * (f32x2){hreg[j][2], hreg[j][3]};
+            rhbuf[(2 * w + j) * 64 + lane] = (f32x4){rh_lo.x, rh_lo.y, rh_hi.x, rh_hi.y};
+        }
+#pragma unroll
+        for (int j = 0; j < 2; ++j) {
+            const f32x2 u_lo = sigmoid2((f32x2){acc_u[j][0], acc_u[j][1]});
+            const f32x2 u_hi = sigmoid2((f32x2){acc_u[j][2], acc_u[j][3]});
+            u[j] = (f32x4){u_lo.x, u_lo.y, u_hi.x, u_hi.y};
+        }
+#pragma unroll
+        for (int j = 0; j < 2; ++j) { acc_r[j] = bias_r[j]; acc_u[j] = bias_u[j]; }
+        __builtin_amdgcn_sched_barrier(0);
+        gates_x_part(xcur, k_lo{}, k_mid{}, pinned{});
+        lds_barrier();
+        hb_a = rhbuf[0 * 64 + lane];
+        hb_b = rhbuf[1 * 64 + lane];
+        group_commit();
+        gates_x_part(xcur, k_mid{}, k_hi{}, pinned{});
+
+        resident_prefence(acc_c[0], acc_c[1]);
+#pragma unroll
+        for (int nn = 0; nn < NT; ++nn) {
+            const f32x4 rb = (nn & 1) ? hb_b : hb_a;
+            if (nn + 2 < NT) {
+                if (nn & 1) hb_b = rhbuf[(nn + 2) * 64 + lane]; else hb_a = rhbuf[(nn + 2) * 64 + lane];
+            }
+            __builtin_amdgcn_sched_barrier(0);
+#pragma unroll
+            for (int e = 0; e < 4; ++e) {
+                const int kc = 4 * nn + e;
+                const float rv = rb[e];
+                KWS_MFMA_A(acc_c[0], wch[0][kc], rv);
+                KWS_MFMA_A(acc_c[1], wch[1][kc], rv);
+            }
+        }
+        resident_fence(acc_c[0], acc_c[1]);
+        const unsigned live = t < len_s ? 0xffffffffu : 0u;
+        f32x4 hout[2];
+#pragma unroll
+        for (int j = 0; j < 2; ++j) {
+#pragma unroll
+            for (int h2 = 0; h2 < 2; ++h2) {
+                const f32x2 c = tanh2((f32x2){acc_c[j][2 * h2], acc_c[j][2 * h2 + 1]});
+                const f32x2 uu = {u[j][2 * h2], u[j][2 * h2 + 1]};
+                const f32x2 hh = {hreg[j][2 * h2], hreg[j][2 * h2 + 1]};
+                const f32x2 hn = (1.0f - uu) * c + uu * hh;
+                hreg[j][2 * h2] = bitsel(live, hn.x, hh.x);
+                hreg[j][2 * h2 + 1] = bitsel(live, hn.y, hh.y);
+                if (LAST) {
+                    hout[j][2 * h2] = bitsel(live, hn.x, 0.f);
+                    hout[j][2 * h2 + 1] = bitsel(live, hn.y, 0.f);
+                }
+            }
+        }
+#pragma unroll
+        for (int j = 0; j < 2; ++j) acc_c[j] = bias_c[j];
+        constexpr int NCX = 2 * KCX;
+        constexpr int NPOST = NCX >= 32 ? 16 : 8;
+        constexpr int NPRE = NCX - NPOST;
+        auto cand_x_mfma = [&](auto mc) {
+            constexpr int m = decltype(mc)::value, kc = m / 2;
+            if constexpr (m % 2 == 0) acc_c[0] = mfma4(wcx[0][kc], xcur[kc], acc_c[0]);
+            else acc_c[1] = mfma4(wcx[1][kc], xcur[kc], acc_c[1]);
+        };
+        if constexpr (FIRST) {
+            coop_commit();
+            if constexpr (kIssueAtEnd) coop_issue(t + 3);
+        }
+#pragma unroll
+        for (int j = 0; j < 2; ++j) {
+            hbuf[(2 * w + j) * 64 + lane] = hreg[j];
+            if (!LAST) {
+                const f32x4 o = hreg[j];
+                p.h_out[((size_t)group * T + t) * NT * 64 + (2 * w + j) * 64 + lane] =
+                    make_float4(o[0], o[1], o[2], o[3]);
+            }
+        }
+        if (LAST) {
+            f32x4 accf = bfc4;
+#pragma unroll
+            for (int j = 0; j < 2; ++j)
+#pragma unroll
+                for (int e = 0; e < 4; ++e) accf = mfma4(wfc[j][e], hout[j][e], accf);
+            if (g < 2) *reinterpret_cast<f32x4*>(epi.pstage + (w * 16 + s) * 8 + 4 * g) = accf;
+        }
+        __builtin_amdgcn_sched_barrier(0);
+        static_for<0, NPRE>(cand_x_mfma);
+        __builtin_amdgcn_sched_barrier(0);
+        lds_barrier();
+        hb_a = hbuf[0 * 64 + lane];
+        hb_b = hbuf[1 * 64 + lane];
+        FoldRegs fold;
+        const bool folder = LAST && w == (t & 3);
+        if (folder) epilogue_fold_load(epi, lane, fold);
+        __builtin_amdgcn_sched_barrier(0);
+        static_for<NPRE, NCX>(cand_x_mfma);
+        __builtin_amdgcn_sched_barrier(0);
+        if (LAST) {
+            if (folder) epilogue_fold_store(epi, t, lane, fold);
+            if (((t + 1) & (kRingFrames - 1)) == 0 || t == T - 1) {
+                const int t0 = t & ~(kRingFrames - 1);
+                lds_barrier();
+                epilogue_flush(p, epi, group, t0, t - t0 + 1, w, lane, t == T - 1);
+            }
+        }
+    };
+
+    for (; group < n_groups; group += gridDim.x) {
+    enter_group();
+    if constexpr (!FIRST) {
+        if (T > 0) {
+            group_issue(1);
+#pragma unroll
+            for (int sl = 0; sl < NT; ++sl) load_x_slice(xbuf0, 0, sl);
+            group_commit();
+        }
+    }
+    __syncthreads();
+    if (T > 0) {
+        if constexpr (FIRST) {
+            coop_issue(0);
+            coop_commit();
+            __syncthreads();
+            read_xs(xbuf0);
+            coop_issue(1);
+        }
+#pragma unroll
+        for (int j = 0; j < 2; ++j) { acc_r[j] = bias_r[j]; acc_u[j] = bias_u[j]; }
+        gates_x_part(xbuf0, k_lo{}, k_hi{}, pinned{});
+        hb_a = hbuf[0 * 64 + lane];
+        hb_b = hbuf[1 * 64 + lane];
+        cand_x(xbuf0);
+        if constexpr (FIRST) {
+            __syncthreads();
+            coop_commit();
+            if constexpr (kIssueAtEnd) coop_issue(2);
+            __syncthreads();
+        }
+    }
+    for (int t = 0; t < T; ++t) frame(t, xbuf0, xbuf0);
+
+    if (bvalid) {
+#pragma unroll
+        for (int j = 0; j < 2; ++j)
+            *reinterpret_cast<f32x4*>(p.state_out + (size_t)b * H + (2 * w + j) * 16 + 4 * g) = hreg[j];
+    }
+    __syncthreads();
+    if constexpr (WINDOW) {
+        const WindowTail win = window_tail_params_from_kernarg(kWinOffset);
+        WindowTailRegs<2> wreq;
+        window_tail_request<2>(win, p.B, group * kStreamsPerGroup, tid, wreq);
+        window_tail<2>(win, p.B, group * kStreamsPerGroup, T, epi.cwords, kWinTailWordsStride, win_dl, reinterpret_cast<char*>(hbuf), tid, wreq);
+        __syncthreads();
+    }
+    }
+}
+
+int gru_resident_kcx(int in_dim, bool first) { return first ? (in_dim + 3) / 4 : 32; }
+
+bool gru_resident_supported(int hidden, int in_dim, bool first) {
+    if (hidden != 128) return false;
+    if (!first) return in_dim == 128;
+    return in_dim == 32 || in_dim == 40 || in_dim == 48 || in_dim == 60 || in_dim == 64;
+}
+
+bool gru_resident_takes_window(bool first, bool last) { return last && !first; }
+
+hipError_t launch_gru_layer_resident(const GruLayerParams& p, bool first, bool last, hipStream_t st) {
+    const size_t lds = resident_lds_bytes(p.KCX, first, last);
+    const dim3 grid(persistent_grid(p.B));
+    if (p.win.tab != nullptr) {
+        if (!gru_resident_takes_window(first, last) || p.seq_len) return hipErrorInvalidValue;
+        return launch_lds<gru_layer_resident<32, false, true, true>>(grid, dim3(256), lds + kWinTailWordsBytes, st, p);
+    }
+    return with_bool(last, [&](auto la) {
+        if (!first) return launch_lds<gru_layer_resident<32, false, la()>>(grid, dim3(256), lds, st, p);
+        return with_int<8, 10, 12, 15, 16>(p.KCX, [&](auto kcx) {
+            return launch_lds<gru_layer_resident<kcx(), true, la()>>(grid, dim3(256), lds, st, p);
+        });
+    });
+}
+
+}
```

Result: faster. 399.7 million, median of 6 (+2.5%).
